# Kalyan0821/ecnf-baseline-neurips-2023

Measured on NVIDIA B200. Metric: LJ13 samples/s with exact log-q (Dopri5), higher is better.
Workload: dtype f32

## Files before the change

ecnf_b200/csrc/ecnf_solve_impl.cuh:

```cuda
#pragma once
#include <cstdio>

#include "ecnf_solve_decl.cuh"
#include "ecnf_tile.cuh"

namespace ecnf_solve_detail {

using ecnf_tile::NTHREADS;
using ecnf_tile::WCHUNK;
using ecnf_tile::ColT;
using ecnf_tile::tile_gemm;

enum { KIND_FIRST = 0, KIND_MID = 1, KIND_LAST = 2 };

static __constant__ float c_A[7][6] = {
    {0, 0, 0, 0, 0, 0},
    {(float)(1.0 / 5), 0, 0, 0, 0, 0},
    {(float)(3.0 / 40), (float)(9.0 / 40), 0, 0, 0, 0},
    {(float)(44.0 / 45), (float)(-56.0 / 15), (float)(32.0 / 9), 0, 0, 0},
    {(float)(19372.0 / 6561), (float)(-25360.0 / 2187), (float)(64448.0 / 6561), (float)(-212.0 / 729), 0, 0},
    {(float)(9017.0 / 3168), (float)(-355.0 / 33), (float)(46732.0 / 5247), (float)(49.0 / 176),
     (float)(-5103.0 / 18656), 0},
    {(float)(35.0 / 384), 0, (float)(500.0 / 1113), (float)(125.0 / 192), (float)(-2187.0 / 6784),
     (float)(11.0 / 84)}};
static __constant__ float c_C[7] = {0.f, 0.2f, 0.3f, 0.8f, (float)(8.0 / 9), 1.f, 1.f};
static __constant__ float c_BERR[7] = {(float)(35.0 / 384 - 1951.0 / 21600),
                                0.f,
                                (float)(500.0 / 1113 - 22642.0 / 50085),
                                (float)(125.0 / 192 - 451.0 / 720),
                                (float)(-2187.0 / 6784 + 12231.0 / 42400),
                                (float)(11.0 / 84 - 649.0 / 6300),
                                (float)(-1.0 / 60)};
static __constant__ float c_MID[7] = {(float)(6025192743.0 / 30085553152.0 / 2),
                               0.f,
                               (float)(51252292925.0 / 65400821598.0 / 2),
                               (float)(-2691868925.0 / 45128329728.0 / 2),
                               (float)(187940372067.0 / 1594534317056.0 / 2),
                               (float)(-1776094331.0 / 19743644256.0 / 2),
                               (float)(11237099.0 / 235043384.0 / 2)};

template <int U_, int H_>
struct Geo {
  static constexpr int U = U_, H = H_;
  static constexpr int TR = (U_ == 256) ? 64 : 128;
  static constexpr int LD = U_ + 4;
  static constexpr int RT = TR / 16;
  static constexpr int GMAX = TR / 3 + 1;
};

struct SmemLayout {
  int X1, X2, Wb, G, xt, xtacc, dacc, xs, xs0, xacc, mu, rowdot, rowsd, gv, gs1, glen, ginv, ge, tau, cvec,
      ode, red, rowslot, rowgrp, gi, gj, giz, epsv, total_floats;
};

template <int U, int H>
__host__ __device__ inline SmemLayout make_layout(int n, int dim, bool div) {
  using G_ = Geo<U, H>;
  const int D = n * dim, S = D + 1;
  SmemLayout L;
  int o = 0;
  auto take = [&](int nfl) { int r = o; o += (nfl + 3) & ~3; return r; };
  L.X1 = take(G_::TR * G_::LD);
  L.X2 = take(G_::TR * G_::LD);
  L.Wb = take(2 * WCHUNK);
  L.G = take(div ? G_::GMAX * U : 4);
  L.xt = take(div ? D * D : 4);
  L.xtacc = take(div ? D * D : 4);
  L.dacc = take(D);
  L.xs = take(D);
  L.xs0 = take(D);
  L.xacc = take(D);
  L.mu = take(4);
  L.rowdot = take(G_::TR);
  L.rowsd = take(G_::TR);
  L.gv = take(G_::TR * 3);
  L.gs1 = take(G_::TR);
  L.glen = take(G_::TR);
  L.ginv = take(G_::TR);
  L.ge = take(G_::TR);
  L.tau = take(ECNF_MAX_T);
  L.cvec = take(64);
  L.ode = take(11 * S);
  L.red = take(S + 16);
  L.rowslot = take(G_::TR);
  L.rowgrp = take(G_::TR);
  L.gi = take(G_::TR);
  L.gj = take(G_::TR);
  L.giz = take(G_::TR);
  L.epsv = take(D);
  L.total_floats = o;
  return L;
}

template <int N, int TR, int LD>
__device__ __forceinline__ void epi_act(float (&acc)[TR / 16][ColT<N>::CT], const float* __restrict__ bias,
                                        float* dst, int nrows, int r, const int* rowgrp, float* G, bool has_tan) {
  constexpr int RT = TR / 16, CT = ColT<N>::CT, NSEG = CT / 4;
  const int tid = threadIdx.x, tx = tid & 15, ty = tid >> 4, warp = tid >> 5;
  const bool active = (2 * RT * warp < nrows) && (tx * 4 < N);
  const int row0 = 2 * RT * warp + (ty & 1);
  if (active) {
#pragma unroll
    for (int rr = 0; rr < RT; ++rr) {
      const int row = row0 + 2 * rr;
      if (row >= nrows) continue;
      const int g = rowgrp[row];
      if (row != g * r) continue;
#pragma unroll
      for (int sg = 0; sg < NSEG; ++sg) {
        const int col = sg * 64 + tx * 4;
        const float4 b = *reinterpret_cast<const float4*>(bias + col);
        const float bb[4] = {b.x, b.y, b.z, b.w};
        float a[4], gg[4];
#pragma unroll
        for (int q = 0; q < 4; ++q) {
          const float z = acc[rr][4 * sg + q] + bb[q];
          const float s = ecnf_sigmoid(z);
          a[q] = z * s;
          gg[q] = s * (1.f + z * (1.f - s));
        }
        *reinterpret_cast<float4*>(dst + row * LD + col) = make_float4(a[0], a[1], a[2], a[3]);
        if (has_tan) *reinterpret_cast<float4*>(G + g * N + col) = make_float4(gg[0], gg[1], gg[2], gg[3]);
      }
    }
  }
  if (has_tan) {
    __syncthreads();
    if (active) {
#pragma unroll
      for (int rr = 0; rr < RT; ++rr) {
        const int row = row0 + 2 * rr;
        if (row >= nrows) continue;
        const int g = rowgrp[row];
        if (row == g * r) continue;
#pragma unroll
        for (int sg = 0; sg < NSEG; ++sg) {
          const int col = sg * 64 + tx * 4;
          const float4 gg = *reinterpret_cast<const float4*>(G + g * N + col);
          *reinterpret_cast<float4*>(dst + row * LD + col) =
              make_float4(acc[rr][4 * sg] * gg.x, acc[rr][4 * sg + 1] * gg.y, acc[rr][4 * sg + 2] * gg.z,
                          acc[rr][4 * sg + 3] * gg.w);
        }
      }
    }
  }
  __syncthreads();
}

template <int N, int TR, int LD>
__device__ __forceinline__ void epi_linear(float (&acc)[TR / 16][ColT<N>::CT], const float* bias, float* dst,
                                           int nrows, int r, const int* rowgrp, const float* resid) {
  constexpr int RT = TR / 16, CT = ColT<N>::CT, NSEG = CT / 4;
  const int tid = threadIdx.x, tx = tid & 15, ty = tid >> 4, warp = tid >> 5;
  const bool active = (2 * RT * warp < nrows) && (tx * 4 < N);
  const int row0 = 2 * RT * warp + (ty & 1);
  if (active) {
#pragma unroll
    for (int rr = 0; rr < RT; ++rr) {
      const int row = row0 + 2 * rr;
      if (row >= nrows) continue;
      const bool primal = (row == rowgrp[row] * r);
#pragma unroll
      for (int sg = 0; sg < NSEG; ++sg) {
        const int col = sg * 64 + tx * 4;
        float v[4] = {acc[rr][4 * sg], acc[rr][4 * sg + 1], acc[rr][4 * sg + 2], acc[rr][4 * sg + 3]};
        if (bias != nullptr && primal) {
#pragma unroll
          for (int q = 0; q < 4; ++q) v[q] += bias[col + q];
        }
        if (resid != nullptr) {
          const float4 rv = *reinterpret_cast<const float4*>(resid + row * LD + col);
          v[0] += rv.x; v[1] += rv.y; v[2] += rv.z; v[3] += rv.w;
        }
        *reinterpret_cast<float4*>(dst + row * LD + col) = make_float4(v[0], v[1], v[2], v[3]);
      }
    }
  }
  __syncthreads();
}

__device__ __forceinline__ int dirmap(int kind, int qq, int i, int j, int dim) {
  if (kind == KIND_MID) return qq;
  if (kind == KIND_LAST) return i * dim + qq;
  return (qq < dim) ? i * dim + qq : j * dim + (qq - dim);
}


template <int U, int H, bool DIV>
struct Engine {
  using G_ = Geo<U, H>;
  static constexpr int TR = G_::TR, LD = G_::LD, RT = G_::RT;
  static constexpr int NT = NTHREADS;
  const EcnfModelDev& m;
  const bool hutch;
  const int n, dim, D, ntan, ND, E;
  const int tid;
  const float* eps_g;
  float *X1, *X2, *Wb, *G, *xt, *xtacc, *dacc, *xs, *xs0, *xacc, *mu, *rowdot, *rowsd, *gv, *gs1, *glen, *ginv,
      *ge, *tau, *cvec, *ode, *red, *epsv;
  int *rowslot, *rowgrp, *gi, *gj, *giz;
  float *hA, *hB, *Ps, *Pr, *Mg;

  __device__ Engine(const EcnfModelDev& m_, float* smem, float* scratch, bool hutch_)
      : m(m_), hutch(DIV && hutch_), n(m_.n), dim(m_.dim), D(m_.n * m_.dim),
        ntan(DIV ? (hutch_ ? 1 : m_.n * m_.dim) : 0), ND(1 + ntan), E(m_.n * (m_.n - 1)), tid(threadIdx.x), eps_g(nullptr) {
    const SmemLayout L = make_layout<U, H>(n, dim, DIV);
    X1 = smem + L.X1; X2 = smem + L.X2; Wb = smem + L.Wb; G = smem + L.G; xt = smem + L.xt;
    xtacc = smem + L.xtacc; dacc = smem + L.dacc; xs = smem + L.xs; xs0 = smem + L.xs0; xacc = smem + L.xacc;
    mu = smem + L.mu; rowdot = smem + L.rowdot; rowsd = smem + L.rowsd; gv = smem + L.gv; gs1 = smem + L.gs1;
    glen = smem + L.glen; ginv = smem + L.ginv; ge = smem + L.ge; tau = smem + L.tau; cvec = smem + L.cvec;
    ode = smem + L.ode; red = smem + L.red; epsv = smem + L.epsv;
    rowslot = reinterpret_cast<int*>(smem + L.rowslot); rowgrp = reinterpret_cast<int*>(smem + L.rowgrp);
    gi = reinterpret_cast<int*>(smem + L.gi); gj = reinterpret_cast<int*>(smem + L.gj);
    giz = reinterpret_cast<int*>(smem + L.giz);
    hA = scratch; hB = hA + (size_t)n * ND * H; Ps = hB + (size_t)n * ND * H; Pr = Ps + (size_t)n * ND * U;
    Mg = Pr + (size_t)n * ND * U;
  }

  __device__ __forceinline__ void set_eps(const float* e) { eps_g = e; }
  __device__ __forceinline__ float* ode_ptr() const { return ode; }
  __device__ __forceinline__ float* red_ptr() const { return red; }

  __device__ void rowdot_tile(const float* X, const float* __restrict__ vec, int nrows) {
    const int warp = tid >> 5, lane = tid & 31;
    float v[U / 32];
#pragma unroll
    for (int j = 0; j < U / 32; ++j) v[j] = vec[lane + 32 * j];
    for (int row = warp; row < nrows; row += NTHREADS / 32) {
      float s = 0.f;
#pragma unroll
      for (int j = 0; j < U / 32; ++j) s = fmaf(X[row * LD + lane + 32 * j], v[j], s);
#pragma unroll
      for (int o = 16; o > 0; o >>= 1) s += __shfl_xor_sync(0xffffffffu, s, o);
      if (lane == 0) rowdot[row] = s;
    }
    __syncthreads();
  }

  template <int W>
  __device__ void store_node_tile(const float* X, float* dst, int node0, int nrows, int r) {
    for (int idx = tid; idx < nrows * (W / 4); idx += NTHREADS) {
      const int row = idx / (W / 4), c4 = idx % (W / 4);
      const int g = row / r, q = row - g * r;
      *reinterpret_cast<float4*>(dst + ((size_t)(node0 + g) * ND + q) * W + c4 * 4) =
          *reinterpret_cast<const float4*>(X + row * LD + c4 * 4);
    }
  }
  template <int W>
  __device__ void load_node_tile(float* X, const float* src, int node0, int nrows, int r, bool tan_valid) {
    for (int idx = tid; idx < nrows * (W / 4); idx += NTHREADS) {
      const int row = idx / (W / 4), c4 = idx % (W / 4);
      const int g = row / r, q = row - g * r;
      float4 v = make_float4(0.f, 0.f, 0.f, 0.f);
      if (q == 0 || tan_valid) v = *reinterpret_cast<const float4*>(src + ((size_t)(node0 + g) * ND + q) * W + c4 * 4);
      *reinterpret_cast<float4*>(X + row * LD + c4 * 4) = v;
    }
  }
  __device__ void set_rowgrp(int nrows, int r) {
    for (int row = tid; row < nrows; row += NTHREADS) rowgrp[row] = row / r;
  }

  __device__ void node_pre(int b, bool htan) {
    const EcnfBlockParams& bp = m.blk[b];
    if (tid < H) {
      float a = bp.bd[tid];
      for (int k = 0; k < m.T; ++k) a = fmaf(tau[k], bp.Wd[(H + k) * H + tid], a);
      cvec[tid] = a;
    }
    const int r = htan ? ND : 1;
    const int gpt = TR / r;
    for (int node0 = 0; node0 < n; node0 += gpt) {
      const int nn = min(gpt, n - node0), nrows = nn * r;
      __syncthreads();
      load_node_tile<H>(X1, hA, node0, nrows, r, true);
      set_rowgrp(nrows, r);
      __syncthreads();
      {
        float acc[RT][ColT<H>::CT];
        tile_gemm<H, H, TR, LD, true>(X1, bp.Wd, Wb, acc, nrows);
        epi_linear<H, TR, LD>(acc, cvec, X2, nrows, r, rowgrp, nullptr);
      }
      store_node_tile<H>(X2, hB, node0, nrows, r);
      {
        float acc[RT][ColT<U>::CT];
        tile_gemm<H, U, TR, LD, true>(X2, bp.We[0], Wb, acc, nrows);
        epi_linear<U, TR, LD>(acc, nullptr, X1, nrows, r, rowgrp, nullptr);
        store_node_tile<U>(X1, Ps, node0, nrows, r);
        tile_gemm<H, U, TR, LD, true>(X2, bp.We[0] + (size_t)H * U, Wb, acc, nrows);
        epi_linear<U, TR, LD>(acc, bp.be[0], X1, nrows, r, rowgrp, nullptr);
        store_node_tile<U>(X1, Pr, node0, nrows, r);
      }
    }
    __syncthreads();
  }

  __device__ void node_post(int b, bool htan) {
    const EcnfBlockParams& bp = m.blk[b];
    const int r = ND;
    const int gpt = TR / r;
    for (int node0 = 0; node0 < n; node0 += gpt) {
      const int nn = min(gpt, n - node0), nrows = nn * r;
      __syncthreads();
      load_node_tile<U>(X1, Mg, node0, nrows, r, true);
      load_node_tile<H>(X2, hB, node0, nrows, r, htan);
      set_rowgrp(nrows, r);
      __syncthreads();
      {
        float acc[RT][ColT<U>::CT];
        tile_gemm<U, U, TR, LD, true>(X1, bp.Wh[0], Wb, acc, nrows);
        tile_gemm<H, U, TR, LD, false>(X2, bp.Wh[0] + (size_t)U * U, Wb, acc, nrows);
        epi_act<U, TR, LD>(acc, bp.bh[0], X1, nrows, r, rowgrp, G, DIV);
        for (int l = 1; l < m.L; ++l) {
          tile_gemm<U, U, TR, LD, true>(X1, bp.Wh[l], Wb, acc, nrows);
          epi_act<U, TR, LD>(acc, bp.bh[l], X1, nrows, r, rowgrp, G, DIV);
        }
      }
      {
        float acc[RT][ColT<H>::CT];
        tile_gemm<U, H, TR, LD, true>(X1, bp.Wh[m.L], Wb, acc, nrows);
        epi_linear<H, TR, LD>(acc, bp.bh[m.L], X1, nrows, r, rowgrp, X2);
      }
      store_node_tile<H>(X1, hA, node0, nrows, r);
    }
    __syncthreads();
  }

  __device__ void edge_phase(int b, int kind, bool htan, bool lastb) {
    const EcnfBlockParams& bp = m.blk[b];
    const int nact = !DIV ? 0 : (kind == KIND_MID ? ntan : kind == KIND_LAST ? dim : 2 * dim);
    const int r = 1 + nact;
    const int gpt = DIV ? min(TR / r, n - 1) : TR;
    const float inv_sqrt_nb = rsqrtf((float)(n - 1));
    const float* wd = bp.We[0] + (size_t)2 * H * U;
    const float bpv = bp.bp[0];
    const float bav = bp.ba[0];
    for (int i = tid; i < D; i += NTHREADS) { xacc[i] = 0.f; dacc[i] = 0.f; }
    if (DIV && kind != KIND_LAST)
      for (int i = tid; i < D * ntan; i += NTHREADS) xtacc[i] = 0.f;
    if (!lastb)
      for (int i = tid; i < n * ND * U; i += NTHREADS) Mg[i] = 0.f;
    __syncthreads();

    int e0 = 0;
    while (e0 < E) {
      int ng;
      if (DIV) {
        const int i = e0 / (n - 1);
        ng = min(gpt, (i + 1) * (n - 1) - e0);
      } else {
        ng = min(TR, E - e0);
      }
      const int nrows = ng * r;
      if (tid < ng) {
        const int e = e0 + tid, i = e / (n - 1), jj = e - i * (n - 1);
        int j = i + 1 + jj; if (j >= n) j -= n;
        float s = 0.f;
        for (int c = 0; c < dim; ++c) {
          const float v = xs[i * dim + c] - xs[j * dim + c];
          gv[tid * 3 + c] = v;
          s = fmaf(v, v, s);
        }
        const int isz = (s == 0.f);
        const float s1 = isz ? 1.f : s;
        const float len = sqrtf(s1);
        gi[tid] = i; gj[tid] = j; giz[tid] = isz; gs1[tid] = s1; glen[tid] = len; ginv[tid] = 1.f / (m.C + len);
      }
      __syncthreads();
      for (int row = tid; row < nrows; row += NTHREADS) {
        const int g = row / r, q = row - g * r;
        rowgrp[row] = g;
        if (q == 0) {
          rowslot[row] = 0;
          rowsd[row] = gs1[g];
        } else {
          const int i = gi[g], j = gj[g];
          const int k = dirmap(kind, q - 1, i, j, dim);
          float sd = 0.f;
          for (int c = 0; c < dim; ++c)
            sd = fmaf(gv[g * 3 + c], xt[(i * dim + c) * ntan + k] - xt[(j * dim + c) * ntan + k], sd);
          rowslot[row] = 1 + k;
          rowsd[row] = giz[g] ? 0.f : 2.f * sd;
        }
      }
      __syncthreads();
      {
        const int col = tid % U;
        const float wdc = wd[col];
        for (int g = tid / U; g < ng; g += NTHREADS / U) {
          const int row = g * r;
          const float z = Ps[((size_t)gj[g] * ND) * U + col] + Pr[((size_t)gi[g] * ND) * U + col] + rowsd[row] * wdc;
          const float s = ecnf_sigmoid(z);
          X1[row * LD + col] = z * s;
          if (DIV) G[g * U + col] = s * (1.f + z * (1.f - s));
        }
        if (DIV) {
          __syncthreads();
          for (int row = tid / U; row < nrows; row += NTHREADS / U) {
            const int g = rowgrp[row];
            if (row == g * r) continue;
            float z = rowsd[row] * wdc;
            if (htan) {
              const int slot = rowslot[row];
              z += Ps[((size_t)gj[g] * ND + slot) * U + col] + Pr[((size_t)gi[g] * ND + slot) * U + col];
            }
            X1[row * LD + col] = z * G[g * U + col];
          }
        }
      }
      __syncthreads();
      {
        float acc[RT][ColT<U>::CT];
        for (int l = 1; l < m.L; ++l) {
          tile_gemm<U, U, TR, LD, true>(X1, bp.We[l], Wb, acc, nrows);
          epi_act<U, TR, LD>(acc, bp.be[l], X1, nrows, r, rowgrp, G, DIV);
        }
        if (!lastb) {
          rowdot_tile(X1, bp.wa, nrows);
          if (tid < ng) ge[tid] = ecnf_sigmoid(rowdot[tid * r] + bav);
          __syncthreads();
          for (int idx = tid; idx < nrows * U; idx += NTHREADS) {
            const int row = idx / U, col = idx - row * U;
            const int g = rowgrp[row];
            const float e = ge[g];
            float v = X1[row * LD + col] * e;
            if (row != g * r) v = fmaf(X1[g * r * LD + col], e * (1.f - e) * rowdot[row], v);
            X2[row * LD + col] = v;
          }
          __syncthreads();
          if (DIV) {
            const int i = gi[0];
            for (int idx = tid; idx < r * U; idx += NTHREADS) {
              const int q = idx / U, col = idx - q * U;
              const bool shared_q = (q == 0) || kind == KIND_MID || (q - 1 < dim);
              if (shared_q) {
                const int slot = (q == 0) ? 0 : 1 + dirmap(kind, q - 1, i, 0, dim);
                float s = 0.f;
                for (int g = 0; g < ng; ++g) s += X2[(g * r + q) * LD + col];
                Mg[((size_t)i * ND + slot) * U + col] += s * inv_sqrt_nb;
              } else {
                for (int g = 0; g < ng; ++g) {
                  const int slot = 1 + gj[g] * dim + (q - 1 - dim);
                  Mg[((size_t)i * ND + slot) * U + col] += X2[(g * r + q) * LD + col] * inv_sqrt_nb;
                }
              }
            }
          } else {
            const int i_first = e0 / (n - 1), i_last = (e0 + ng - 1) / (n - 1);
            for (int idx = tid; idx < (i_last - i_first + 1) * U; idx += NTHREADS) {
              const int ri = idx / U, col = idx - ri * U, i = i_first + ri;
              const int ga = max(e0, i * (n - 1)) - e0, gb = min(e0 + ng, (i + 1) * (n - 1)) - e0;
              float s = 0.f;
              for (int g = ga; g < gb; ++g) s += X2[g * LD + col];
              Mg[(size_t)i * U + col] += s * inv_sqrt_nb;
            }
          }
        }
        for (int l = 0; l < m.L; ++l) {
          tile_gemm<U, U, TR, LD, true>(X1, bp.Wx[l], Wb, acc, nrows);
          epi_act<U, TR, LD>(acc, bp.bx[l], X1, nrows, r, rowgrp, G, DIV);
        }
      }
      rowdot_tile(X1, bp.wp, nrows);
      {
        const int i_first = e0 / (n - 1), i_last = (e0 + ng - 1) / (n - 1);
        const int nprim = (i_last - i_first + 1) * dim;
        const int nwork_tan = DIV ? (r - 1) * dim : 0;
        for (int idx = tid; idx < nprim + nwork_tan; idx += NTHREADS) {
          if (idx < nprim) {
            const int ri = idx / dim, c = idx - ri * dim, i = i_first + ri;
            const int ga = max(e0, i * (n - 1)) - e0, gb = min(e0 + ng, (i + 1) * (n - 1)) - e0;
            float s = 0.f;
            for (int g = ga; g < gb; ++g) s = fmaf((rowdot[g * r] + bpv) * gv[g * 3 + c], ginv[g], s);
            xacc[i * dim + c] += s;
          } else {
            const int t2 = idx - nprim;
            const int q = 1 + t2 / dim, c = t2 % dim;
            const int i = gi[0];
            for (int g = 0; g < ng; ++g) {
              const int j = gj[g];
              const int k = dirmap(kind, q - 1, i, j, dim);
              if (kind == KIND_LAST && k != i * dim + c) continue;
              const float pg = rowdot[g * r] + bpv, pd = rowdot[g * r + q];
              const float vc = gv[g * 3 + c], inv = ginv[g];
              const float vd = xt[(i * dim + c) * ntan + k] - xt[(j * dim + c) * ntan + k];
              const float ld = giz[g] ? 0.f : rowsd[g * r + q] / (2.f * glen[g]);
              const float cd = (pd * vc + pg * vd) * inv - pg * vc * ld * inv * inv;
              if (kind == KIND_LAST) dacc[i * dim + c] += cd;
              else xtacc[(i * dim + c) * ntan + k] += cd;
            }
          }
        }
      }
      __syncthreads();
      e0 += ng;
    }
  }

  __device__ void eval(float t, const float* xin, const int32_t* feat, float* fout) {
    if (tid < dim) {
      float s = 0.f;
      for (int i = 0; i < n; ++i) s += xin[i * dim + tid];
      mu[tid] = s / (float)n;
    }
    if (tid >= 32 && tid < 32 + m.T / 2) {
      const int k = tid - 32;
      const float arg = (t * 1000.f) * m.freqs[k];
      tau[k] = sinf(arg);
      tau[k + m.T / 2] = cosf(arg);
    }
    __syncthreads();
    for (int i = tid; i < D; i += NTHREADS) {
      const float v = xin[i] - mu[i % dim];
      xs[i] = v;
      xs0[i] = v;
    }
    if (DIV && !hutch) {
      const float invn = 1.f / (float)n;
      for (int idx = tid; idx < D * D; idx += NTHREADS) {
        const int a = idx / D, k = idx - a * D;
        const int ia = a / dim, ca = a - ia * dim, ik = k / dim, ck = k - ik * dim;
        xt[idx] = (ca == ck) ? ((ia == ik ? 1.f : 0.f) - invn) : 0.f;
      }
    }
    if (hutch) {
      for (int i = tid; i < D; i += NTHREADS) epsv[i] = eps_g[i];
      __syncthreads();
      for (int i = tid; i < D; i += NTHREADS) {
        float mean = 0.f;
        for (int node = 0; node < n; ++node) mean += epsv[node * dim + i % dim];
        xt[i] = epsv[i] - mean / (float)n;
      }
    }
    for (int idx = tid; idx < n * H; idx += NTHREADS) {
      const int node = idx / H, col = idx - node * H;
      int f = feat[node];
      f = max(0, min(m.nfeat - 1, f));
      hA[(size_t)node * ND * H + col] = m.embed[f * H + col];
    }
    __syncthreads();
    for (int b = 0; b < m.nblocks; ++b) {
      const bool last = (b == m.nblocks - 1);
      const int kind = hutch ? KIND_MID : (last ? KIND_LAST : (b == 0 ? KIND_FIRST : KIND_MID));
      const bool htan = DIV && b > 0;
      node_pre(b, htan);
      edge_phase(b, kind, htan, last);
      if (!last) node_post(b, htan);
      const float invnb = 1.f / (float)(n - 1);
      for (int i = tid; i < D; i += NTHREADS) xs[i] += xacc[i] * invnb;
      if (DIV && (!last || hutch))
        for (int i = tid; i < D * ntan; i += NTHREADS) xt[i] += xtacc[i] * invnb;
      __syncthreads();
    }
    const float fs = m.final_scaling[0];
    for (int i = tid; i < D; i += NTHREADS) fout[i] = (xs[i] - xs0[i] - mu[i % dim]) * fs;
    if (DIV && tid == 0) {
      float s = 0.f;
      if (hutch) {
        for (int d = 0; d < D; ++d) s = fmaf(epsv[d], xt[d] - epsv[d], s);
        fout[D] = fs * s;
      } else {
        const float invnb = 1.f / (float)(n - 1);
        for (int d = 0; d < D; ++d) s += xt[d * D + d] + dacc[d] * invnb;
        fout[D] = fs * (s - (float)D);
      }
    }
    __syncthreads();
  }
};

__device__ __forceinline__ float clip_to_end(float tprev, float tnext, float T1, bool keep) {
  if (tnext > T1 - 1e-6f) return keep ? T1 : tprev + 0.5f * (T1 - tprev);
  return tnext;
}

template <class Eng, bool DIV, bool SAVE>
__device__ __forceinline__ void solve_body(const KernelArgs& a, Eng& eng, long long& s_traj, float* s_ctl) {
  const int tid = threadIdx.x;
  const int D = eng.D, S = DIV ? D + 1 : D;
  float* y = eng.ode_ptr();
  float* ys = y + S;
  float* f0 = ys + S;
  float* fo = f0 + S;
  float* kk = fo + S;
  float* red = eng.red_ptr();
  const ecnf_solve_ctrl& c = a.ctrl;
  const bool vf_mode = (a.mode == ECNF_MODE_VF || a.mode == ECNF_MODE_VF_DIV);
  const bool reverse = (a.mode == ECNF_MODE_LOGPROB);
  const float dir = reverse ? -1.f : 1.f;
  const float T0 = reverse ? -1.f : 0.f, T1 = reverse ? 0.f : 1.f;
  enum { PH_VF = 0, PH_F0 = 1, PH_F1 = 2, PH_STAGE = 3 };

  auto rms_of_red = [&]() -> float {
    __syncthreads();
    if (tid == 0) {
      float s = 0.f;
      for (int i = 0; i < S; ++i) s = fmaf(red[i], red[i], s);
      s_ctl[0] = sqrtf(s / (float)S);
    }
    __syncthreads();
    const float r = s_ctl[0];
    __syncthreads();
    return r;
  };
  auto base_logp = [&](const float* v) -> float {
    __syncthreads();
    if (tid == 0) {
      float s = 0.f;
      for (int cdim = 0; cdim < eng.dim; ++cdim) {
        float mean = 0.f;
        for (int i = 0; i < eng.n; ++i) mean += v[i * eng.dim + cdim] / a.m.base_scale;
        mean /= (float)eng.n;
        for (int i = 0; i < eng.n; ++i) {
          const float z = v[i * eng.dim + cdim] / a.m.base_scale - mean;
          s = fmaf(z, z, s);
        }
      }
      const float dof = (float)((eng.n - 1) * eng.dim);
      s_ctl[1] = -0.5f * s - 0.5f * dof * 1.8378770664093453f - dof * logf(a.m.base_scale);
    }
    __syncthreads();
    const float r = s_ctl[1];
    __syncthreads();
    return r;
  };

  for (;;) {
    if (tid == 0) s_traj = (long long)atomicAdd(a.counter, 1u);
    __syncthreads();
    const long long b = s_traj;
    __syncthreads();
    if (b >= a.B) break;
    const int32_t* feat = a.feat + b * eng.n;
    const float* xin = a.x_init + b * D;
    eng.set_eps(a.eps ? a.eps + b * D : nullptr);
    auto put = [&](int k, int i, float v) {
      if (i < D) a.out_traj[(b * a.n_save + k) * D + i] = v;
      else a.out_traj_delta[b * a.n_save + k] = v;
    };
    int next_save = 0;

    int phase, stage = 0, n_steps = 0, n_acc = 0, n_evals = 0, status = 0;
    float tprev = T0, tnext = T0, dt = 0.f, h0 = 0.f, d1 = 0.f, t_eval, lp0_start = 0.f;
    bool at_dtmin = false;
    const float* ein;
    if (vf_mode) {
      for (int i = tid; i < D; i += Eng::NT) ys[i] = xin[i];
      phase = PH_VF;
      t_eval = a.t_in[b];
      ein = ys;
    } else {
      for (int i = tid; i < S; i += Eng::NT) y[i] = (i < D) ? xin[i] : 0.f;
      phase = PH_F0;
      t_eval = dir * T0;
      ein = y;
    }
    __syncthreads();
    if constexpr (SAVE) {
      for (; next_save < a.n_save && a.ts[next_save] <= T0; ++next_save)
        for (int i = tid; i < S; i += Eng::NT) put(next_save, i, y[i]);
    }
    if (DIV && !vf_mode && !reverse) lp0_start = base_logp(y);

    bool running = true;
    while (running) {
      eng.eval(t_eval, ein, feat, fo);
      ++n_evals;
      bool begin_step = false;
      if (phase == PH_VF) {
        for (int i = tid; i < D; i += Eng::NT) a.out_x[b * D + i] = fo[i];
        if (DIV && tid == 0) a.out_logs[b] = fo[D];
        running = false;
      } else if (phase == PH_F0) {
        for (int i = tid; i < S; i += Eng::NT) f0[i] = dir * fo[i];
        __syncthreads();
        if (c.fixed) {
          tnext = clip_to_end(tprev, tprev + fabsf(c.step_size), T1, true);
          begin_step = true;
        } else {
          for (int i = tid; i < S; i += Eng::NT) red[i] = y[i] / (c.atol + fabsf(y[i]) * c.rtol);
          const float d0 = rms_of_red();
          for (int i = tid; i < S; i += Eng::NT) red[i] = f0[i] / (c.atol + fabsf(y[i]) * c.rtol);
          d1 = rms_of_red();
          const bool cond = (d0 < 1e-5f) || (d1 < 1e-5f);
          h0 = cond ? 1e-6f : 0.01f * d0 / d1;
          for (int i = tid; i < S; i += Eng::NT) ys[i] = y[i] + h0 * f0[i];
          __syncthreads();
          t_eval = dir * (tprev + h0);
          ein = ys;
          phase = PH_F1;
        }
      } else if (phase == PH_F1) {
        for (int i = tid; i < S; i += Eng::NT) red[i] = (dir * fo[i] - f0[i]) / (c.atol + fabsf(y[i]) * c.rtol);
        const float d2 = rms_of_red() / h0;
        const float md = fmaxf(d1, d2);
        const float h1 = (md <= 1e-15f) ? fmaxf(1e-6f, h0 * 1e-3f) : powf(0.01f / md, 1.f / c.error_order);
        const float dt0 = fmaxf(fminf(100.f * h0, h1), c.dtmin);
        tnext = clip_to_end(tprev, tprev + dt0, T1, true);
        begin_step = true;
      } else {
        for (int i = tid; i < S; i += Eng::NT) kk[stage * S + i] = (dir * fo[i]) * dt;
        __syncthreads();
        if (stage < 6) {
          ++stage;
        } else {
          bool keep = true;
          float new_prev, new_next;
          if (c.fixed) {
            new_prev = tnext;
            new_next = tnext + dt;
          } else {
            for (int i = tid; i < S; i += Eng::NT) {
              float e = 0.f;
              for (int j = 0; j < 7; ++j) {
                const float bj = c_BERR[j];
                if (bj != 0.f) e = e + bj * kk[j * S + i];
              }
              red[i] = (c.err_scale * e) / (c.atol + fmaxf(fabsf(y[i]), fabsf(ys[i])) * c.rtol);
            }
            const float err = rms_of_red();
            keep = (err < 1.f) || at_dtmin;
            const float inv = (err == 0.f) ? INFINITY : 1.f / err;
            float factor = c.safety * powf(inv, 1.f / c.error_order);
            const float fmin_ = keep ? 1.f : c.factormin;
            factor = fminf(fmaxf(factor, fmin_), c.factormax);
            float ndt = dt * factor;
            at_dtmin = ndt <= c.dtmin;
            ndt = fmaxf(ndt, c.dtmin);
            new_prev = keep ? tnext : tprev;
            new_next = new_prev + ndt;
          }
          new_prev = fminf(new_prev, T1);
          new_next = clip_to_end(new_prev, new_next, T1, keep);
          if constexpr (SAVE) {
            for (; keep && next_save < a.n_save && a.ts[next_save] <= tnext; ++next_save) {
              const float tau_s = a.ts[next_save];
              const bool at_end = !(tau_s < tnext);
              const float sx = (tau_s - tprev) / dt;
              for (int i = tid; i < S; i += Eng::NT) {
                const float y0 = y[i], y1 = ys[i];
                float v = y1;
                if (!at_end) {
                  const float k0 = kk[i], k6 = kk[6 * S + i];
                  float ym = y0;
                  for (int j = 0; j < 7; ++j) {
                    const float cj = c_MID[j];
                    if (cj != 0.f) ym = ym + cj * kk[j * S + i];
                  }
                  const float pa = 2.f * (k6 - k0) - 8.f * (y1 + y0) + 16.f * ym;
                  const float pb = 5.f * k0 - 3.f * k6 + 18.f * y0 + 14.f * y1 - 32.f * ym;
                  const float pc = k6 - 4.f * k0 - 11.f * y0 - 5.f * y1 + 16.f * ym;
                  v = (((pa * sx + pb) * sx + pc) * sx + k0) * sx + y0;
                }
                put(next_save, i, v);
              }
            }
          }
          if (keep) {
            for (int i = tid; i < S; i += Eng::NT) { y[i] = ys[i]; f0[i] = dir * fo[i]; }
            ++n_acc;
          }
          __syncthreads();
          tprev = new_prev;
          tnext = new_next;
          ++n_steps;
          if (!(tprev < T1)) running = false;
          else if (n_steps >= c.max_steps) { status = 1; running = false; }
          else begin_step = true;
        }
      }
      if (begin_step) {
        dt = tnext - tprev;
        for (int i = tid; i < S; i += Eng::NT) kk[i] = f0[i] * dt;
        __syncthreads();
        stage = 1;
        phase = PH_STAGE;
        if (c.max_steps <= 0) { status = 1; running = false; }
      }
      if (running && phase == PH_STAGE) {
        for (int i = tid; i < S; i += Eng::NT) {
          float v = y[i];
          for (int j = 0; j < stage; ++j) {
            const float aj = c_A[stage][j];
            if (aj != 0.f) v = v + aj * kk[j * S + i];
          }
          ys[i] = v;
        }
        __syncthreads();
        t_eval = dir * (tprev + c_C[stage] * dt);
        ein = ys;
      }
    }
    if (vf_mode) { __syncthreads(); continue; }
    if constexpr (SAVE) {
      const int left = a.n_save - next_save;
      for (int idx = tid; idx < left * S; idx += Eng::NT) put(next_save + idx / S, idx % S, __int_as_float(0x7fffffff));
    }

    for (int i = tid; i < D; i += Eng::NT) a.out_x[b * D + i] = y[i];
    float lpb_end = 0.f;
    if (DIV && reverse) lpb_end = base_logp(y);
    if (tid == 0) {
      if (a.out_stats) {
        a.out_stats[b * 4 + 0] = n_steps; a.out_stats[b * 4 + 1] = n_acc;
        a.out_stats[b * 4 + 2] = n_evals; a.out_stats[b * 4 + 3] = status;
      }
      if (DIV && a.out_logs) {
        const float delta = y[D];
        if (!reverse) {
          a.out_logs[b * 3 + 0] = lp0_start - delta;
          a.out_logs[b * 3 + 1] = lp0_start;
          a.out_logs[b * 3 + 2] = delta;
        } else {
          a.out_logs[b * 3 + 0] = lpb_end + delta;
          a.out_logs[b * 3 + 1] = lpb_end;
          a.out_logs[b * 3 + 2] = delta;
        }
      }
    }
    __syncthreads();
  }
}

template <int U, int H, bool DIV, bool SAVE>
__global__ void __launch_bounds__(NTHREADS, 1) ecnf_solve_kernel(const __grid_constant__ KernelArgs a) {
  extern __shared__ __align__(16) float smem[];
  __shared__ long long s_traj;
  __shared__ float s_ctl[8];
  Engine<U, H, DIV> eng(a.m, smem, a.scratch + (size_t)blockIdx.x * a.scratch_stride, a.eps != nullptr);
  solve_body<Engine<U, H, DIV>, DIV, SAVE>(a, eng, s_traj, s_ctl);
}

template <int U, int H, bool DIV>
int simt_check(const ecnf_model* mdl) {
  const SmemLayout L = make_layout<U, H>(mdl->cfg.n_frames, mdl->cfg.dim, DIV);
  const size_t smem = (size_t)L.total_floats * sizeof(float);
  if (smem > 227 * 1024) {
    ecnf_set_error("shared memory need %zu B exceeds 227 KB (n_frames=%d dim=%d U=%d)", smem, mdl->cfg.n_frames,
                   mdl->cfg.dim, U);
    return ECNF_ERR_UNSUPPORTED;
  }
  if (DIV && 1 + mdl->cfg.n_frames * mdl->cfg.dim > Geo<U, H>::TR) {
    ecnf_set_error("1 + n_frames*dim = %d tangent slots exceed the %d-row tile of U=%d", 1 + mdl->cfg.n_frames * mdl->cfg.dim,
                   Geo<U, H>::TR, U);
    return ECNF_ERR_UNSUPPORTED;
  }
  return ECNF_OK;
}

template <int U, int H, bool DIV, bool SAVE>
int launch_t(const ecnf_model* mdl, KernelArgs& a, int grid, cudaStream_t st) {
  const int rc = simt_check<U, H, DIV>(mdl);
  if (rc != ECNF_OK) return rc;
  const size_t smem = (size_t)make_layout<U, H>(mdl->cfg.n_frames, mdl->cfg.dim, DIV).total_floats * sizeof(float);
  auto kern = ecnf_solve_kernel<U, H, DIV, SAVE>;
  ECNF_CHECK_CUDA(cudaFuncSetAttribute(kern, cudaFuncAttributeMaxDynamicSharedMemorySize, (int)smem));
  kern<<<grid, NTHREADS, smem, st>>>(a);
  ECNF_CHECK_CUDA(cudaGetLastError());
  return ECNF_OK;
}


}
```

ecnf_b200/csrc/ecnf_solve_tc.cuh:

```cuda
#pragma once
#include "ecnf_solve_impl.cuh"
#include "ecnf_tc.cuh"

namespace ecnf_solve_detail {

using namespace ecnf_tc;

constexpr int TC_NT = 384;
constexpr int TC_EPI = 256, TC_SIDE = 96;
#ifndef TC_WPREFETCH
#define TC_WPREFETCH 0
#endif
constexpr int TC_BOP = 65536;
constexpr uint32_t TC_LBO = 128, TC_SBO = 2048;
constexpr uint32_t TC_LBO_K = 2048, TC_SBO_K = 128;
constexpr int TC_WCOL = 256;

constexpr uint32_t CH_VALID = 1u << 31, CH_GRPEND = 1u << 22, CH_OWNER = 1u << 23, CH_RUNEND = 1u << 24;
__host__ __device__ __forceinline__ int ch_gid(uint32_t w) { return (int)(w & 1023u); }
__host__ __device__ __forceinline__ int ch_qb(uint32_t w) { return (int)((w >> 10) & 255u); }
__host__ __device__ __forceinline__ int ch_cnt(uint32_t w) { return (int)((w >> 18) & 15u); }
enum { TH_N = 0, TH_FLUSH, TH_WIN_I, TH_WIN_NR, TH_WIN_S, TH_WIN_NS, TH_NCH , TH_IFIRST = 10, TH_ILAST, TH_P, TH_MR, TH_RUNMASK };

__device__ __forceinline__ float fast_sigmoid(float z) {
  float e, r;
  asm("ex2.approx.ftz.f32 %0, %1;" : "=f"(e) : "f"(z * -1.4426950408889634f));
  asm("rcp.approx.ftz.f32 %0, %1;" : "=f"(r) : "f"(1.f + e));
  return r;
}
__device__ __forceinline__ float2 fast_sigmoid2(float2 z) {
  const float2 t = mul2(z, splat2(-1.4426950408889634f));
  float2 e, r;
  asm("ex2.approx.ftz.f32 %0, %1;" : "=f"(e.x) : "f"(t.x));
  asm("ex2.approx.ftz.f32 %0, %1;" : "=f"(e.y) : "f"(t.y));
  const float2 d = add2(splat2(1.f), e);
  asm("rcp.approx.ftz.f32 %0, %1;" : "=f"(r.x) : "f"(d.x));
  asm("rcp.approx.ftz.f32 %0, %1;" : "=f"(r.y) : "f"(d.y));
  return r;
}
__device__ __forceinline__ float2 col2(const float (&v)[64], int c) { return make_float2(v[c], v[c + 1]); }
__device__ __forceinline__ void set_col2(float (&v)[64], int c, float2 p) { v[c] = p.x; v[c + 1] = p.y; }

__host__ __device__ inline int tc_rows_of_kind(int kind, int n, int dim, int ntan) {
  const int ND = 1 + ntan;
  return (kind == TT_NODE1 || kind == TT_EDGE1) ? 1 : kind == TT_NODE ? ND : kind == TT_FIRST ? 1 + 2 * dim : kind == TT_MID ? ND : 1 + dim;
}

__host__ __device__ inline int tc_pack(int kind, int n, int dim, int SUB, int MR, uint32_t* out, int ntan, uint32_t* stage = nullptr) {
  const int ND = 1 + ntan, nb = n - 1;
  const bool edge = kind >= TT_FIRST;
  const int ngroups = edge ? n * nb : n;
  const int r = tc_rows_of_kind(kind, n, dim, ntan);
  const bool dense = (r == 1);
  const int CAP = 16 * SUB;
  int tile = 0, p = 0;
  int win_i = 0, win_nr = 0, win_s = 0, win_ns = 0, i_first = 0, i_last = 0;
  int run_start = 0;
  auto tp = [&](int t) { return stage ? stage : out + (size_t)t * TC_TILE_WORDS; };
  auto word_index = [&](int q) { return (q % SUB) * 16 + ((q / SUB) % 2) * 8 + q / (2 * SUB); };
  auto end_run = [&](bool each_chunk = false) {
    if (out && p > run_start) {
      tp(tile)[word_index(p - 1)] |= CH_RUNEND;
      for (int q = run_start; q < p; ++q)
        if (each_chunk || q + 2 * SUB >= p) tp(tile)[word_index(q)] |= CH_GRPEND;
    }
    run_start = p;
  };
  auto close = [&](int flush) {
    if (p == 0) return;
    end_run();
    if (out) {
      uint32_t* h = tp(tile) + 32;
      int nmax0 = 0, nmax1 = 0;
      for (int sb = 0; sb < SUB; ++sb)
        for (int hh = 0; hh < 2; ++hh) {
          const int first = sb + SUB * hh;
          const int cntp = p > first ? (p - first + 2 * SUB - 1) / (2 * SUB) : 0;
          h[TH_NCH + sb * 2 + hh] = (uint32_t)cntp;
          if (hh == 0 && cntp > nmax0) nmax0 = cntp;
          if (hh == 1 && cntp > nmax1) nmax1 = cntp;
        }
      int N = nmax1 > 0 ? 64 + 8 * nmax1 : 8 * nmax0;
      N = (N + 15) & ~15;
      h[TH_N] = (uint32_t)(N < 16 ? 16 : N);
      h[TH_FLUSH] = (uint32_t)flush;
      h[TH_WIN_I] = (uint32_t)win_i; h[TH_WIN_NR] = (uint32_t)win_nr; h[TH_WIN_S] = (uint32_t)win_s; h[TH_WIN_NS] = (uint32_t)win_ns;
      h[TH_IFIRST] = (uint32_t)i_first; h[TH_ILAST] = (uint32_t)i_last; h[TH_P] = (uint32_t)p; h[TH_MR] = (uint32_t)MR;
      uint32_t rm = 0u;
      for (int q = 0; q < p; ++q)
        if (tp(tile)[word_index(q)] & CH_RUNEND) rm |= 1u << q;
      h[TH_RUNMASK] = rm;
      if (stage)
        for (int k = 0; k < TC_TILE_WORDS; ++k) out[(size_t)tile * TC_TILE_WORDS + k] = stage[k];
    }
    ++tile;
    p = 0; run_start = 0;
  };
  auto put = [&](int gid, int qb, int cnt, bool owner) {
    if (p == CAP) close(0);
    if (p == 0 && out)
      for (int k = 0; k < TC_TILE_WORDS; ++k) tp(tile)[k] = 0;
    const int i = edge ? gid / nb : gid;
    if (p == 0) i_first = i;
    i_last = edge ? (gid + (dense ? cnt - 1 : 0)) / nb : gid + (dense ? cnt - 1 : 0);
    if (out)
      tp(tile)[word_index(p)] = CH_VALID | (uint32_t)gid | ((uint32_t)qb << 10) | ((uint32_t)cnt << 18) | (owner ? CH_OWNER : 0u);
    ++p;
  };
  if (dense) {
    win_i = 0; win_nr = n; win_s = 0; win_ns = 1;
    for (int g = 0; g < ngroups; g += 8) {
      put(g, 0, ngroups - g < 8 ? ngroups - g : 8, true);
      end_run();
    }
    close(kind == TT_EDGE1 ? 1 : 0);
    return tile;
  }
  if (kind == TT_NODE) {
    for (int g = 0; g < n; ++g)
      for (int qb = 1; qb < r; qb += 7) { put(g, qb, 1 + (r - qb < 7 ? r - qb : 7), qb == 1); end_run(); }
    close(0);
    return tile;
  }
  if (kind == TT_LAST) {
    for (int i = 0; i < n; ++i) {
      for (int e = i * nb; e < (i + 1) * nb; ++e) {
        if (p == CAP) close(0);
        put(e, 1, r, true);
      }
      end_run();
    }
    close(0);
    return tile;
  }
  if (kind == TT_FIRST) {
    const int rows_per = 1 + dim;
    int W = MR / rows_per; if (W < 1) W = 1; if (W > n) W = n;
    for (int i0 = 0; i0 < n; i0 += W) {
      win_i = i0; win_nr = (n - i0 < W) ? n - i0 : W; win_s = 0; win_ns = rows_per;
      for (int i = i0; i < i0 + win_nr; ++i) {
        for (int e = i * nb; e < (i + 1) * nb; ++e) {
          if (p == CAP) { end_run(true); close(0); }
          put(e, 1, r, true);
        }
        end_run(true);
      }
      close(1);
    }
    return tile;
  }
  if (ND <= MR) {
    int W = MR / ND; if (W > n) W = n;
    for (int i0 = 0; i0 < n; i0 += W) {
      win_i = i0; win_nr = (n - i0 < W) ? n - i0 : W; win_s = 0; win_ns = ND;
      for (int i = i0; i < i0 + win_nr; ++i)
        for (int qb = 1; qb < r; qb += 7) {
          for (int e = i * nb; e < (i + 1) * nb; ++e) {
            if (p == CAP) close(0);
            put(e, qb, 1 + (r - qb < 7 ? r - qb : 7), qb == 1);
          }
          end_run();
        }
      close(1);
    }
  } else {
    const int cpw = (MR - 1) / 7 > 0 ? (MR - 1) / 7 : 1;
    for (int i = 0; i < n; ++i)
      for (int qw = 1; qw < r; qw += 7 * cpw) {
        const int q_end = (qw + 7 * cpw < r) ? qw + 7 * cpw : r;
        win_i = i; win_nr = 1; win_s = (qw == 1) ? 0 : qw; win_ns = q_end - win_s;
        for (int qb = qw; qb < q_end; qb += 7) {
          for (int e = i * nb; e < (i + 1) * nb; ++e) {
            if (p == CAP) close(0);
            put(e, qb, 1 + (r - qb < 7 ? r - qb : 7), qb == 1);
          }
          end_run();
        }
        close(1);
      }
  }
  return tile;
}

template <int U, int H>
__host__ __device__ inline TcSmemLayout make_tc_layout(int n, int dim, int MR) {
  constexpr int SUB = 128 / U;
  const int D = n * dim, S = D + 1, E = n * (n - 1);
  TcSmemLayout L;
  int o = 0;
  auto take = [&](int bytes) { int r = o; o += (bytes + 127) & ~127; return r; };
  L.bop = take(2 * TC_BOP);
  L.mrows = MR;
  L.macc = take(2 * SUB * (MR + 1) * U * 4);
  L.xt = take(D * D * 4);
  L.xtacc = take(D * D * 4);
  L.dacc = take(D * 4);
  L.xs = take(D * 4);
  L.xs0 = take(D * 4);
  L.xacc = take(D * 4);
  L.mu = take(16);
  L.tau = take(ECNF_MAX_T * 4);
  L.cvec = take(64 * 4);
  L.ode = take(11 * S * 4);
  L.red = take((S + 16) * 4);
  L.colsd = take(4 * SUB * 128 * 4);
  L.colmrow = take(4 * SUB * 128 * 4);
  L.chw = take(4 * 32 * 4);
  L.hdr = take(4 * 16 * 4);
  L.pdot = take(2 * 8 * 64 * 4);
  L.pdh = take(4 * 8 * 64 * 4);
  L.wA = take(8 * 64 * 4);
  L.wB = take(8 * 64 * 4);
  L.cdbuf = take(SUB * 128 * 3 * 4);
  L.egv = take(E * 4 * 4);
  L.bars = take(128);
  L.prof = take(32 * 8);
  L.total_bytes = o;
  return L;
}
template <int U, int H>
__host__ inline int tc_pick_mrows(int n, int dim, bool div) {
  const int ND = div ? 1 + n * dim : 1;
  if (!div) return n;
  int best = 0;
  const int cap = ND > 40 ? ND : 40;
  for (int mr = 8; mr <= cap; ++mr) {
    if (mr < ND && (mr - 1) % 7 != 0) continue;
    if (make_tc_layout<U, H>(n, dim, mr).total_bytes + 1024 <= 227 * 1024) best = mr;
  }
  return best;
}

extern __shared__ __align__(1024) unsigned char smem_tc[];

#define TCF(field) (reinterpret_cast<float*>(smem_tc + a.lay.field))
#define TCI(field) (reinterpret_cast<int*>(smem_tc + a.lay.field))
#define TCW(field) (reinterpret_cast<uint32_t*>(smem_tc + a.lay.field))

template <int U_, int H_, bool DIV>
struct EngineTC {
  static constexpr int U = U_, H = H_, SUB = 128 / U_;
  static constexpr int NT = TC_NT;
  static constexpr int KN = SUB * H;
  static constexpr int ROWB = 4 * H;
  const KernelArgs& a;
  const EcnfModelDev& m;
  const TcImages& img;
  const bool hutch;
  const int n, dim, D, ntan, ND, E;
  const float* eps_g;
  const int tid, f, hh, warp, lane, sub, fu;
  const bool is_epi, is_side;
  uint32_t tmem;
  uint32_t lane_addr;
  uint32_t par;

  enum { B_READY = 0, B_DONE = 1, B_BUILT = 2, B_HEADS = 3, B_BFREE = 4 };
  enum { P_NODE_PRE, P_EDGE, P_NODE_POST, P_WAIT, P_EPI, P_MSG, P_HEAD, P_WLOAD, P_SIDE_WAIT, P_SIDE_GATHER, P_SIDE_COORD,
         P_SIDE_META, P_SIDE_CPWAIT, P_NBUILD, P_NCOUNT };
#ifdef ECNF_TC_PROFILE
  long long prof_t0, prof_t1;
  __device__ __forceinline__ long long* prof_s() const { return reinterpret_cast<long long*>(smem_tc + a.lay.prof); }
  __device__ __forceinline__ void pbeg() { prof_t0 = clock64(); }
  __device__ __forceinline__ void pend(int k) { const long long t1 = clock64(); if (tid == 0) prof_s()[k] += t1 - prof_t0; prof_t0 = t1; }
  __device__ __forceinline__ void qbeg() { prof_t1 = clock64(); }
  __device__ __forceinline__ void qend(int k) { const long long t1 = clock64(); if (tid == 0 || tid == TC_EPI) prof_s()[k] += t1 - prof_t1; prof_t1 = t1; }
#else
  __device__ __forceinline__ void pbeg() {}
  __device__ __forceinline__ void pend(int) {}
  __device__ __forceinline__ void qbeg() {}
  __device__ __forceinline__ void qend(int) {}
#endif

  __device__ __forceinline__ void set_eps(const float* e) { eps_g = e; }
  __device__ __forceinline__ float* ode_ptr() const { return TCF(ode); }
  __device__ __forceinline__ float* red_ptr() const { return TCF(red); }
  __device__ __forceinline__ uint64_t* bar(int kind, int s) const { return reinterpret_cast<uint64_t*>(smem_tc + a.lay.bars) + kind * 2 + s; }
  __device__ __forceinline__ uint32_t* tmem_slot() const { return reinterpret_cast<uint32_t*>(smem_tc + a.lay.bars + 96); }
  __device__ __forceinline__ float* hA() const { return a.scratch + (size_t)blockIdx.x * a.scratch_stride; }
  __device__ __forceinline__ float* hB() const { return hA() + (size_t)n * ND * H; }
  __device__ __forceinline__ float* Mg() const { return hB() + (size_t)n * ND * H; }
  __device__ __forceinline__ float* Ph() const { return Mg() + (size_t)n * ND * U; }
  __device__ __forceinline__ unsigned char* Himg() const { return reinterpret_cast<unsigned char*>(Ph() + (size_t)n * ND * U); }

  __device__ __forceinline__ EngineTC(const KernelArgs& a_)
      : a(a_), m(a_.m), img(a_.img), hutch(DIV && a_.eps != nullptr), n(a_.m.n), dim(a_.m.dim), D(a_.m.n * a_.m.dim),
        ntan(DIV ? (a_.eps != nullptr ? 1 : a_.m.n * a_.m.dim) : 0), ND(1 + (DIV ? (a_.eps != nullptr ? 1 : a_.m.n * a_.m.dim) : 0)),
        E(a_.m.n * (a_.m.n - 1)), eps_g(nullptr), tid(threadIdx.x), f(threadIdx.x & 127), hh((threadIdx.x >> 7) & 1), warp(threadIdx.x >> 5),
        lane(threadIdx.x & 31), sub((threadIdx.x & 127) / U_), fu((threadIdx.x & 127) % U_), is_epi(threadIdx.x < TC_EPI),
        is_side(threadIdx.x >= TC_EPI && threadIdx.x < TC_EPI + TC_SIDE) {
    if (tid == 0) {
      mbar_init(bar(B_READY, 0), TC_EPI); mbar_init(bar(B_READY, 1), TC_EPI);
      mbar_init(bar(B_DONE, 0), 1); mbar_init(bar(B_DONE, 1), 1);
      mbar_init(bar(B_BUILT, 0), TC_SIDE); mbar_init(bar(B_BUILT, 1), TC_SIDE);
      mbar_init(bar(B_HEADS, 0), TC_EPI); mbar_init(bar(B_HEADS, 1), TC_EPI);
      mbar_init(bar(B_BFREE, 0), 1); mbar_init(bar(B_BFREE, 1), 1);
#ifdef ECNF_TC_PROFILE
      for (int k = 0; k < P_NCOUNT; ++k) prof_s()[k] = 0;
#endif
    }
    __syncwarp();
    if (warp == 0) tmem_alloc(tmem_slot(), 512);
    tc_fence_before();
    __syncthreads();
    tc_fence_after();
    tmem = *tmem_slot();
    lane_addr = (uint32_t)(32 * (warp & 3)) << 16;
    par = 0;
    if (is_epi) {
      uint32_t z[32];
#pragma unroll
      for (int c = 0; c < 32; ++c) z[c] = 0u;
#pragma unroll
      for (int q = 0; q < 4; ++q) tmem_st32(tmem + lane_addr + 128u * hh + 32u * q, z);
      tmem_wait_st();
    }
    if (is_side)
      for (int k = tid - TC_EPI; k < ROWB / 4; k += TC_SIDE) reinterpret_cast<uint32_t*>(Himg() + (size_t)n * ND * ROWB)[k] = 0u;
    tc_fence_before();
    __syncthreads();
    tc_fence_after();
  }
  __device__ __forceinline__ void finish(long long* out) {
#ifdef ECNF_TC_PROFILE
    if (out && tid == 0 && blockIdx.x == 0)
      for (int k = 0; k < P_NCOUNT; ++k) out[k] = prof_s()[k];
#endif
    tc_fence_before();
    __syncthreads();
    if (warp == 0) tmem_dealloc(tmem, 512);
  }

  __device__ __forceinline__ void epi_bar() const { named_bar_sync(1, TC_EPI); }
  __device__ __forceinline__ void half_bar() const { named_bar_sync(2 + hh, TC_EPI / 2); }
  __device__ __forceinline__ void side_bar() const { named_bar_sync(4, TC_SIDE); }
  __device__ __forceinline__ void phase_bar() const { named_bar_sync(5, TC_EPI + TC_SIDE); }
  __device__ __forceinline__ void wait_bar(int kind, int s) {
    const uint32_t bit = 1u << (kind * 2 + s);
    mbar_wait_parked(bar(kind, s), (par & bit) ? 1u : 0u, 20000u);
    par ^= bit;
    tc_fence_after();
  }
  __device__ __forceinline__ void wait_done(int s) { qbeg(); wait_bar(B_DONE, s); qend(P_WAIT); }
  __device__ __forceinline__ void arrive(int kind, int s) {
    fence_proxy_async();
    tc_fence_before();
    mbar_arrive(bar(kind, s));
  }
  __device__ __forceinline__ void issue_mma(int s, int tb, int wait_kind, uint32_t a_col, int K, bool kmajor, bool free_b,
                                            bool drained = false) {
    if (lane == 0) {
      if (drained) wait_bar(B_READY, s);
      wait_bar(wait_kind, s);
      const int N = hdr(tb, TH_N);
      const uint32_t idesc = make_idesc_bf16(128, N) | (kmajor ? 0u : IDESC_B_MN);
      const uint32_t bsm = smem_u32(smem_tc + a.lay.bop) + (uint32_t)s * TC_BOP;
      const uint32_t lbo = kmajor ? TC_LBO_K : TC_LBO, sbo = kmajor ? TC_SBO_K : TC_SBO;
      uint64_t bh = make_sdesc(bsm, lbo, sbo);
      uint64_t bl = make_sdesc(bsm + 32768u, lbo, sbo);
      const uint32_t acc = tmem + 128u * s;
      uint32_t a_hi = tmem + a_col, a_lo = tmem + a_col + (uint32_t)(K >> 1);
      const int nk = K >> 4;
      mma_ts(acc, a_hi, bh, idesc, 0u);
      mma_ts(acc, a_lo, bh, idesc, 1u);
      mma_ts(acc, a_hi, bl, idesc, 1u);
      for (int ks = 1; ks < nk; ++ks) {
        bh += (2u * lbo) >> 4; bl += (2u * lbo) >> 4; a_hi += 8; a_lo += 8;
        mma_ts(acc, a_hi, bh, idesc, 1u);
        mma_ts(acc, a_lo, bh, idesc, 1u);
        mma_ts(acc, a_hi, bl, idesc, 1u);
      }
      mma_commit(bar(B_DONE, s));
      if (free_b) mma_commit(bar(B_BFREE, s));
    }
  }

  __device__ __forceinline__ uint32_t my_acc(int s) const { return tmem + 128u * s + lane_addr + 64u * hh; }
  __device__ __forceinline__ void ld_acc(int s, float (&v)[64]) {
    uint32_t x[32], y[32];
    const uint32_t addr = my_acc(s);
    tmem_ld32(addr, x);
    tmem_ld32(addr + 32u, y);
    tmem_wait_ld();
#pragma unroll
    for (int c = 0; c < 32; ++c) { v[c] = __uint_as_float(x[c]); v[32 + c] = __uint_as_float(y[c]); }
  }
  __device__ __forceinline__ void write_B(int s, const float (&v)[64], int krow) {
    unsigned char* base = smem_tc + a.lay.bop + s * TC_BOP + (8 * hh) * (int)TC_SBO + krow * 16;
#pragma unroll
    for (int g8 = 0; g8 < 8; ++g8) {
      uint32_t h[4], l[4];
#pragma unroll
      for (int p = 0; p < 4; ++p) split_pack(v[8 * g8 + 2 * p], v[8 * g8 + 2 * p + 1], h[p], l[p]);
      *reinterpret_cast<uint4*>(base + g8 * (int)TC_SBO) = make_uint4(h[0], h[1], h[2], h[3]);
      *reinterpret_cast<uint4*>(base + 32768 + g8 * (int)TC_SBO) = make_uint4(l[0], l[1], l[2], l[3]);
    }
  }
  __device__ __forceinline__ void ld_half_issue(int s, int hf, uint32_t (&x)[32]) { tmem_ld32(my_acc(s) + 32u * hf, x); }
  template <bool L0>
  __device__ __forceinline__ void act_half(float (&v)[64], int hf, float bias, int tb, float wdf) {
    const float* sdp = TCF(colsd) + (tb * SUB + sub) * 128 + 64 * hh;
#pragma unroll
    for (int c4 = 0; c4 < 4; ++c4) act_chunk<L0>(v, 4 * hf + c4, bias, sdp, wdf);
  }
  __device__ __forceinline__ void write_half(int s, const float (&v)[64], int hf, int krow) {
    unsigned char* base = smem_tc + a.lay.bop + s * TC_BOP + (8 * hh + 4 * hf) * (int)TC_SBO + krow * 16;
#pragma unroll
    for (int g8 = 0; g8 < 4; ++g8) {
      uint32_t h[4], l[4];
#pragma unroll
      for (int p = 0; p < 4; ++p) split_pack(v[32 * hf + 8 * g8 + 2 * p], v[32 * hf + 8 * g8 + 2 * p + 1], h[p], l[p]);
      *reinterpret_cast<uint4*>(base + g8 * (int)TC_SBO) = make_uint4(h[0], h[1], h[2], h[3]);
      *reinterpret_cast<uint4*>(base + 32768 + g8 * (int)TC_SBO) = make_uint4(l[0], l[1], l[2], l[3]);
    }
  }
  __device__ __forceinline__ static int tb_of(int s, int tile) { return s * 2 + ((tile >> 1) & 1); }
  __device__ __forceinline__ int hdr(int tb, int k) const { return TCI(hdr)[tb * 16 + k]; }
  __device__ __forceinline__ int my_nch(int tb) const { return hdr(tb, TH_NCH + sub * 2 + hh); }
  __device__ __forceinline__ uint32_t my_chw(int tb, int ch) const { return TCW(chw)[tb * 32 + sub * 16 + 8 * hh + ch]; }
  template <bool L0>
  __device__ __forceinline__ void act_rule(float (&v)[64], float bias, int tb, float wdf) {
    const float* sdp = TCF(colsd) + (tb * SUB + sub) * 128 + 64 * hh;
#pragma unroll
    for (int ch = 0; ch < 8; ++ch) act_chunk<L0>(v, ch, bias, sdp, wdf);
  }
  template <bool L0>
  __device__ __forceinline__ static void act_chunk(float (&v)[64], int ch, float bias, const float* sdp, float wdf) {
    const int c0 = 8 * ch;
    if constexpr (L0) {
      const float4 s0 = reinterpret_cast<const float4*>(sdp)[2 * ch], s1 = reinterpret_cast<const float4*>(sdp)[2 * ch + 1];
      const float2 w2 = splat2(wdf);
      set_col2(v, c0, fma2(make_float2(s0.x, s0.y), w2, col2(v, c0)));
      set_col2(v, c0 + 2, fma2(make_float2(s0.z, s0.w), w2, col2(v, c0 + 2)));
      set_col2(v, c0 + 4, fma2(make_float2(s1.x, s1.y), w2, col2(v, c0 + 4)));
      set_col2(v, c0 + 6, fma2(make_float2(s1.z, s1.w), w2, col2(v, c0 + 6)));
    }
    if constexpr (!DIV) {
#pragma unroll
      for (int u = 0; u < 8; u += 2) {
        const float2 z = add2(col2(v, c0 + u), splat2(bias));
        set_col2(v, c0 + u, mul2(z, fast_sigmoid2(z)));
      }
    } else {
      const float z = v[c0] + bias;
      const float sg = fast_sigmoid(z);
      const float cur = sg * (1.f + z * (1.f - sg));
      set_col2(v, c0, mul2(make_float2(z, v[c0 + 1]), make_float2(sg, cur)));
#pragma unroll
      for (int u = 2; u < 8; u += 2) set_col2(v, c0 + u, mul2(col2(v, c0 + u), splat2(cur)));
    }
  }
  template <int W>
  __device__ __forceinline__ void bfly_round(float (&x)[32]) const {
    const bool b = (lane & (W >> 1)) != 0;
#pragma unroll
    for (int i = 0; i < W; ++i) {
      const float keep = b ? x[W + i] : x[i], send = b ? x[i] : x[W + i];
      x[i] = keep + __shfl_xor_sync(0xffffffffu, send, W >> 1);
    }
  }
  __device__ __forceinline__ void warp_dot(const float (&v)[64], float wf, float* pd) {
    float x[32];
    {
      const bool b = (lane & 16) != 0;
      const float2 w2 = splat2(wf);
#pragma unroll
      for (int i = 0; i < 32; i += 2) {
        const float2 lo2 = mul2(col2(v, i), w2), hi2 = mul2(col2(v, 32 + i), w2);
        const float lo[2] = {lo2.x, lo2.y}, hi[2] = {hi2.x, hi2.y};
#pragma unroll
        for (int j = 0; j < 2; ++j) {
          const float keep = b ? hi[j] : lo[j], send = b ? lo[j] : hi[j];
          x[i + j] = keep + __shfl_xor_sync(0xffffffffu, send, 16);
        }
      }
    }
    bfly_round<16>(x);
    bfly_round<8>(x);
    bfly_round<4>(x);
    bfly_round<2>(x);
    *reinterpret_cast<float2*>(pd + 2 * lane) = make_float2(x[0], x[1]);
  }
  __device__ __forceinline__ float full_dot(const float* pd, int h2, int sb, int c) const {
    const float* p4 = pd + (4 * h2) * 64 + c;
    if constexpr (SUB == 1) return (p4[0] + p4[64]) + (p4[128] + p4[192]);
    else return p4[(2 * sb) * 64] + p4[(2 * sb + 1) * 64];
  }
  template <int K>
  __device__ __forceinline__ void fetch_w(int img_off, uint32_t (&wv)[2][K / 4]) {
    constexpr int NC = K / 16;
    const uint4* src = reinterpret_cast<const uint4*>(img.base + img_off);
#pragma unroll
    for (int p = 0; p < 2; ++p)
#pragma unroll
      for (int j = 0; j < NC; ++j) {
        const uint4 q = __ldg(src + (size_t)(p * (K / 8) + hh * NC + j) * 128 + f);
        wv[p][4 * j] = q.x; wv[p][4 * j + 1] = q.y; wv[p][4 * j + 2] = q.z; wv[p][4 * j + 3] = q.w;
      }
  }
  template <int K>
  __device__ __forceinline__ void store_w(const uint32_t (&wv)[2][K / 4], uint32_t col) {
#pragma unroll
    for (int p = 0; p < 2; ++p) {
      const uint32_t addr = tmem + col + lane_addr + (uint32_t)(p * (K / 2) + hh * (K / 4));
      if constexpr (K == 128) tmem_st32(addr, wv[p]);
      else tmem_st16(addr, wv[p]);
    }
    tmem_wait_st();
  }
  template <int K>
  __device__ __forceinline__ void load_w(int img_off, uint32_t col) {
    constexpr int NC = K / 16;
    uint32_t wv[2][K / 4];
    const uint4* src = reinterpret_cast<const uint4*>(img.base + img_off);
#pragma unroll
    for (int p = 0; p < 2; ++p)
#pragma unroll
      for (int j = 0; j < NC; ++j) {
        const uint4 q = __ldg(src + (size_t)(p * (K / 8) + hh * NC + j) * 128 + f);
        wv[p][4 * j] = q.x; wv[p][4 * j + 1] = q.y; wv[p][4 * j + 2] = q.z; wv[p][4 * j + 3] = q.w;
      }
#pragma unroll
    for (int p = 0; p < 2; ++p) {
      const uint32_t addr = tmem + col + lane_addr + (uint32_t)(p * (K / 2) + hh * (K / 4));
      if constexpr (K == 128) tmem_st32(addr, wv[p]);
      else tmem_st16(addr, wv[p]);
    }
    tmem_wait_st();
  }

  __device__ __forceinline__ const uint32_t* tile_ptr(int kind, int tile) const {
    return a.tabs.base + (size_t)(a.tabs.off[kind] + tile) * TC_TILE_WORDS;
  }
  __device__ __forceinline__ bool col_of(uint32_t cw, int c, int& gid, int& q) const {
    const int u = c & 7;
    const bool valid = (cw & CH_VALID) && u < ch_cnt(cw);
    const int qb = ch_qb(cw);
    if (qb == 0) { gid = ch_gid(cw) + u; q = 0; }
    else { gid = ch_gid(cw); q = (u == 0) ? 0 : qb + u - 1; }
    return valid;
  }

  template <class P>
  __device__ __forceinline__ void run_phase(P& p) {
    const int ntiles = p.ntiles, NL = p.NL;
    const int npairs = (ntiles + 1) >> 1;
    const int total_q = npairs * NL;
    if (is_epi || (P::side_build && is_side)) p.prologue();
    if (is_epi && p.stream) {
      load_w<128>(p.wimg(0), TC_WCOL);
      if (total_q > 1) load_w<128>(p.wimg(1 % NL), TC_WCOL + 128);
    }
    if constexpr (P::side_build) {
      if (is_epi || is_side) phase_bar();
    }
    if (is_side) {
      if constexpr (P::side_build) {
#pragma unroll 1
        for (int t0 = 0; t0 < 2 && t0 < ntiles; ++t0) {
          p.side_meta(tb_of(t0, t0), t0);
          p.side_gather(t0, t0);
          cp_async_wait<0>();
          arrive(B_BUILT, t0);
        }
#pragma unroll 1
        for (int t0 = 2; t0 < 4 && t0 < ntiles; ++t0) p.side_meta(tb_of(t0 & 1, t0), t0);
#pragma unroll 1
        for (int pr = 0; pr < npairs; ++pr) {
          qbeg();
#pragma unroll 1
          for (int s = 0; s < 2; ++s) {
            const int tile = 2 * pr + s, ntile = tile + 2;
            if (tile >= ntiles) continue;
            if (ntile < ntiles) {
              wait_bar(B_BFREE, s);
              qend(P_SIDE_WAIT);
              p.side_gather(s, ntile);
              qend(P_SIDE_GATHER);
              cp_async_wait<0>();
              qend(P_SIDE_CPWAIT);
            }
            wait_bar(B_HEADS, s);
            qend(P_SIDE_WAIT);
            if (ntile < ntiles) arrive(B_BUILT, s);
          }
#pragma unroll 1
          for (int s = 0; s < 2; ++s) {
            const int tile = 2 * pr + s;
            if (tile >= ntiles) continue;
            p.side_coords(tb_of(s, tile), tile);
            qend(P_SIDE_COORD);
            if (tile + 4 < ntiles) p.side_meta(tb_of(s, tile + 4), tile + 4);
            qend(P_SIDE_META);
          }
        }
      }
      return;
    }
    const int first_kind = P::side_build ? B_BUILT : B_READY;
#pragma unroll 1
    for (int s = 0; s < 2; ++s) {
      if (s >= ntiles) continue;
      if (is_epi) {
        if constexpr (!P::side_build) { p.build(s, tb_of(s, s), s); arrive(B_READY, s); }
      } else {
        issue_mma(s, tb_of(s, s), first_kind, p.a_col(0, 0), p.K(0), P::side_build, false);
      }
    }
    int q = 0;
#pragma unroll 1
    for (int pr = 0; pr < npairs; ++pr) {
#pragma unroll 1
      for (int w = 0; w < NL; ++w, ++q) {
#pragma unroll 1
        for (int s = 0; s < 2; ++s) {
          const int tile = 2 * pr + s;
          if (tile >= ntiles) continue;
          const bool last_slot = (s == 1) || (tile + 1 >= ntiles);
          const int ntile = tile + 2;
          const int tb = tb_of(s, tile);
          if (is_epi) {
            const bool do_w = p.stream && last_slot && q + 2 < total_q;
#if TC_WPREFETCH
            uint32_t wv[2][32];
            if (do_w) fetch_w<128>(p.wimg((w + 2) % NL), wv);
            wait_done(s);
            if (do_w) { qbeg(); store_w<128>(wv, TC_WCOL + 128 * (q & 1)); qend(P_WLOAD); }
#else
            wait_done(s);
            if (do_w) { qbeg(); load_w<128>(p.wimg((w + 2) % NL), TC_WCOL + 128 * (q & 1)); qend(P_WLOAD); }
#endif
            p.epi(s, tb, tile, w);
            if (w < NL - 1) arrive(B_READY, s);
            else if constexpr (P::side_build) arrive(B_HEADS, s);
            else if (ntile < ntiles) { p.build(s, tb_of(s, ntile), ntile); arrive(B_READY, s); }
          } else {
            if (w < NL - 1)
              issue_mma(s, tb, B_READY, p.a_col(q + 1, w + 1), p.K(w + 1), false, P::side_build && w + 1 == NL - 1 && ntile < ntiles);
            else if (ntile < ntiles)
              issue_mma(s, tb_of(s, ntile), first_kind, p.a_col(q + 1, 0), p.K(0), P::side_build, false, P::side_build);
          }
        }
      }
    }
  }

  __device__ __forceinline__ void node_meta(int tb, int kind, int tile) {
    epi_bar();
    const uint32_t* tp = tile_ptr(kind, tile);
    if (tid < 128) {
#pragma unroll
      for (int sb = 0; sb < SUB; ++sb) {
        const uint32_t cw = __ldg(tp + sb * 16 + (tid >> 3));
        int g, q;
        const bool valid = col_of(cw, tid, g, q);
        TCI(colmrow)[(tb * SUB + sb) * 128 + tid] = valid ? g * ND + q : -1;
      }
    } else if (tid < 128 + 48) {
      const uint32_t w = __ldg(tp + (tid - 128));
      if (tid < 128 + 32) TCW(chw)[tb * 32 + (tid - 128)] = w;
      else TCW(hdr)[tb * 16 + (tid - 160)] = w;
    }
    epi_bar();
  }

  struct NodePre {
    EngineTC& e;
    int b, ntiles, NL, kind;
    static constexpr bool stream = false;
    static constexpr bool side_build = false;
    __device__ __forceinline__ uint32_t a_col(int, int w) const { return TC_WCOL + 64u * w; }
    __device__ __forceinline__ int K(int) const { return KN; }
    __device__ __forceinline__ int wimg(int) const { return 0; }
    __device__ __forceinline__ void prologue() {
      const KernelArgs& a = e.a;
      const EcnfBlockParams& bp = e.m.blk[b];
      const TcImgBlock& ib = e.img.blk[b];
      if (e.tid < H) {
        float cv = bp.bd[e.tid];
        for (int k = 0; k < e.m.T; ++k) cv = fmaf(TCF(tau)[k], bp.Wd[(H + k) * H + e.tid], cv);
        TCF(cvec)[e.tid] = cv;
      }
      e.template load_w<KN>(ib.Wd, TC_WCOL);
      if (NL > 1) e.template load_w<KN>(ib.Wh0h, TC_WCOL + 64);
    }
    __device__ __forceinline__ void build(int s, int tb, int tile) {
      const KernelArgs& a = e.a;
      e.qbeg();
      e.node_meta(tb, kind, tile);
      if (e.fu < H) {
        float v[64];
        const float* src = e.hA() + e.fu;
        const int* ro_ = TCI(colmrow) + (tb * SUB + e.sub) * 128 + 64 * e.hh;
#pragma unroll
        for (int c = 0; c < 64; ++c) {
          const int ro = ro_[c];
          const float x = src[(size_t)(ro >= 0 ? ro : 0) * H];
          v[c] = ro >= 0 ? x : 0.f;
        }
        e.write_B(s, v, e.sub * H + e.fu);
      }
      e.qend(P_NBUILD);
    }
    __device__ __forceinline__ void epi(int s, int tb, int, int w) {
      const KernelArgs& a = e.a;
      const EcnfBlockParams& bp = e.m.blk[b];
      float v[64];
      e.ld_acc(s, v);
      const int* ro_ = TCI(colmrow) + (tb * SUB + e.sub) * 128 + 64 * e.hh;
      if (w == 0) {
        if (e.fu >= H) return;
        const float bias = TCF(cvec)[e.fu];
        float* dst = e.hB() + e.fu;
        unsigned char* himg = e.Himg() + 2 * e.fu;
        const bool dense = (kind == TT_NODE1);
#pragma unroll
        for (int c = 0; c < 64; ++c) {
          const bool pr = dense || (c & 7) == 0;
          v[c] += pr ? bias : 0.f;
          const int ro = ro_[c];
          if (ro >= 0) {
            dst[(size_t)ro * H] = v[c];
            const __nv_bfloat16 hi = __float2bfloat16_rn(v[c]);
            const __nv_bfloat16 lo = __float2bfloat16_rn(v[c] - __bfloat162float(hi));
            *reinterpret_cast<__nv_bfloat16*>(himg + (size_t)ro * ROWB) = hi;
            *reinterpret_cast<__nv_bfloat16*>(himg + (size_t)ro * ROWB + 2 * H) = lo;
          }
        }
        if (NL > 1) e.write_B(s, v, e.sub * H + e.fu);
      } else {
        const float bias = bp.bh[0][e.fu];
        float* dst = e.Ph() + e.fu;
        const bool dense = (kind == TT_NODE1);
#pragma unroll
        for (int c = 0; c < 64; ++c) {
          const bool pr = dense || (c & 7) == 0;
          const int ro = ro_[c];
          if (ro >= 0) dst[(size_t)ro * U] = v[c] + (pr ? bias : 0.f);
        }
      }
    }
  };

  struct NodePost {
    EngineTC& e;
    int b, ntiles, NL, kind;
    bool htan;
    static constexpr bool stream = true;
    static constexpr bool side_build = false;
    __device__ __forceinline__ uint32_t a_col(int q, int) const { return TC_WCOL + 128u * (q & 1); }
    __device__ __forceinline__ int K(int) const { return 128; }
    __device__ __forceinline__ void prologue() {}
    __device__ __forceinline__ int wimg(int w) const {
      const TcImgBlock& ib = e.img.blk[b];
      const int L = e.m.L;
      return w == 0 ? ib.Wh0m : (w < L ? ib.Wh[w] : ib.WhL);
    }
    __device__ __forceinline__ void build(int s, int tb, int tile) {
      const KernelArgs& a = e.a;
      e.qbeg();
      e.node_meta(tb, kind, tile);
      float v[64];
      const float* src = e.Mg() + e.fu;
      const int* ro_ = TCI(colmrow) + (tb * SUB + e.sub) * 128 + 64 * e.hh;
#pragma unroll
      for (int cb = 0; cb < 64; cb += 16) {
#pragma unroll
        for (int u = 0; u < 16; ++u) {
          const int ro = ro_[cb + u];
          const float x = src[(size_t)(ro >= 0 ? ro : 0) * U];
          v[cb + u] = ro >= 0 ? x : 0.f;
        }
      }
      e.write_B(s, v, e.f);
      e.qend(P_NBUILD);
    }
    __device__ __forceinline__ void epi(int s, int tb, int, int w) {
      const KernelArgs& a = e.a;
      const EcnfBlockParams& bp = e.m.blk[b];
      const int L = e.m.L;
      const int* ro_ = TCI(colmrow) + (tb * SUB + e.sub) * 128 + 64 * e.hh;
      float v[64];
      if (w == 0) {
        const float* ph = e.Ph() + e.fu;
        e.ld_acc(s, v);
#pragma unroll
        for (int cb = 0; cb < 64; cb += 16) {
          float pv[16];
#pragma unroll
          for (int u = 0; u < 16; ++u) {
            const int c = cb + u;
            const bool pr = DIV ? ((c & 7) == 0) : true;
            const int ro = ro_[c];
            const bool use = ro >= 0 && (pr || htan);
            const float x = ph[(size_t)(use ? ro : 0) * U];
            pv[u] = use ? x : 0.f;
          }
#pragma unroll
          for (int u = 0; u < 16; ++u) v[cb + u] += pv[u];
        }
        e.template act_rule<false>(v, 0.f, tb, 0.f);
        e.write_B(s, v, e.f);
      } else if (w < L) {
        const float bias = bp.bh[w][e.fu];
        e.ld_acc(s, v);
        e.template act_rule<false>(v, bias, tb, 0.f);
        e.write_B(s, v, e.f);
      } else {
        if (e.fu >= H) return;
        const float bias = bp.bh[L][e.fu];
        const float* hin = e.hB() + e.fu;
        float* dst = e.hA() + e.fu;
        e.ld_acc(s, v);
#pragma unroll
        for (int cb = 0; cb < 64; cb += 16) {
          float hv[16];
#pragma unroll
          for (int u = 0; u < 16; ++u) {
            const int c = cb + u;
            const bool pr = DIV ? ((c & 7) == 0) : true;
            const int ro = ro_[c];
            const bool use = ro >= 0 && (pr || htan);
            const float x = hin[(size_t)(use ? ro : 0) * H];
            hv[u] = (use ? x : 0.f) + (pr ? bias : 0.f);
          }
#pragma unroll
          for (int u = 0; u < 16; ++u) {
            const int ro = ro_[cb + u];
            if (ro >= 0) dst[(size_t)ro * H] = v[cb + u] + hv[u];
          }
        }
      }
    }
  };

  struct EdgePh {
    EngineTC& e;
    int b, ntiles, NL, kind;
    bool htan, want_msg;
    float wdf, waf, wpf;
    static constexpr bool stream = true;
    static constexpr bool side_build = true;
    __device__ __forceinline__ uint32_t a_col(int q, int) const { return TC_WCOL + 128u * (q & 1); }
    __device__ __forceinline__ int K(int) const { return 128; }
    __device__ __forceinline__ int ekind() const { return kind == TT_FIRST ? KIND_FIRST : kind == TT_MID ? KIND_MID : KIND_LAST; }
    __device__ __forceinline__ int wimg(int w) const {
      const TcImgBlock& ib = e.img.blk[b];
      const int L = e.m.L;
      return w == 0 ? ib.We0 : (w < L ? ib.We[w] : ib.Wx[w - L]);
    }
    __device__ __forceinline__ void prologue() {
      const KernelArgs& a = e.a;
      const EcnfBlockParams& bp = e.m.blk[b];
      const int n = e.n, dim = e.dim, D = e.D;
      constexpr int NTH = TC_EPI + TC_SIDE;
      if (e.is_epi) {
        wdf = bp.We[0][(size_t)2 * H * U + e.fu];
        waf = bp.wa[e.fu];
        wpf = bp.wp[e.fu];
      }
      for (int i = e.tid; i < D; i += NTH) { TCF(xacc)[i] = 0.f; TCF(dacc)[i] = 0.f; }
      if (DIV && kind != TT_LAST)
        for (int i = e.tid; i < D * e.ntan; i += NTH) TCF(xtacc)[i] = 0.f;
      if (want_msg)
        for (int i = e.tid; i < 2 * SUB * (a.lay.mrows + 1) * U; i += NTH) TCF(macc)[i] = 0.f;
      for (int ed = e.tid; ed < e.E; ed += NTH) {
        const int i = ed / (n - 1), jj = ed - i * (n - 1);
        int j = i + 1 + jj; if (j >= n) j -= n;
        float vv[3];
        for (int c = 0; c < 3; ++c) vv[c] = c < dim ? TCF(xs)[i * dim + c] - TCF(xs)[j * dim + c] : 0.f;
        reinterpret_cast<float4*>(TCF(egv))[ed] = make_float4(vv[0], vv[1], vv[2], __int_as_float(i | (j << 8)));
      }
    }
    __device__ __forceinline__ float4 edge_geo(int ed, int& i, int& j, float& sq) const {
      const KernelArgs& a = e.a;
      const float4 g = reinterpret_cast<const float4*>(TCF(egv))[ed];
      const int ij = __float_as_int(g.w);
      i = ij & 255; j = ij >> 8;
      sq = fmaf(g.z, g.z, fmaf(g.y, g.y, g.x * g.x));
      return g;
    }

    __device__ __forceinline__ void side_gather(int s, int tile) {
      const KernelArgs& a = e.a;
      const int n = e.n, ND = e.ND;
      const uint32_t* tp = e.tile_ptr(kind, tile);
      const unsigned char* himg = e.Himg();
#pragma unroll 1
      for (int item = e.tid - TC_EPI; item < SUB * 128; item += TC_SIDE) {
        const int sb = item >> 7, c = item & 127;
        unsigned char* bbase = smem_tc + a.lay.bop + s * TC_BOP + (c >> 3) * (int)TC_SBO_K + (c & 7) * 16;
        const uint32_t cw = __ldg(tp + sb * 16 + (c >> 3));
        int ed, q;
        const bool valid = e.col_of(cw, c, ed, q);
        int rs = n * ND, rr = n * ND;
        if (valid && (q == 0 || htan)) {
          const int ij = __float_as_int(TCF(egv)[ed * 4 + 3]);
          const int i = ij & 255, j = ij >> 8;
          const int slot = q == 0 ? 0 : 1 + dirmap(ekind(), q - 1, i, j, e.dim);
          rs = j * ND + slot; rr = i * ND + slot;
        }
        const unsigned char* src_s = himg + (size_t)rs * ROWB;
        const unsigned char* src_r = himg + (size_t)rr * ROWB;
        unsigned char* d0 = bbase + ((sb * 2 * H) >> 3) * (int)TC_LBO_K;
#pragma unroll
        for (int g = 0; g < H / 8; ++g) {
          cp_async16(d0 + g * (int)TC_LBO_K, src_s + 16 * g);
          cp_async16(d0 + 32768 + g * (int)TC_LBO_K, src_s + 2 * H + 16 * g);
          cp_async16(d0 + (H / 8 + g) * (int)TC_LBO_K, src_r + 16 * g);
          cp_async16(d0 + 32768 + (H / 8 + g) * (int)TC_LBO_K, src_r + 2 * H + 16 * g);
        }
      }
      cp_async_commit();
    }
    __device__ __forceinline__ void side_meta(int tb, int tile) {
      const KernelArgs& a = e.a;
      const int sc = e.tid - TC_EPI, n = e.n, dim = e.dim, D = e.D, ND = e.ND;
      const uint32_t* tp = e.tile_ptr(kind, tile);
      const int win_i = (int)__ldg(tp + 32 + TH_WIN_I), win_s = (int)__ldg(tp + 32 + TH_WIN_S), win_ns = (int)__ldg(tp + 32 + TH_WIN_NS);
      const int dump = a.lay.mrows * U;
#pragma unroll 1
      for (int item = sc; item < SUB * 128; item += TC_SIDE) {
        const int sb = item >> 7, c = item & 127;
        const uint32_t cw = __ldg(tp + sb * 16 + (c >> 3));
        int ed, q;
        const bool valid = e.col_of(cw, c, ed, q);
        float sd = 0.f;
        int mr = dump;
        if (valid) {
          int i, j; float sq;
          const float4 g = edge_geo(ed, i, j, sq);
          const float gv[3] = {g.x, g.y, g.z};
          const bool isz = (sq == 0.f);
          int gslot = 0;
          if (q == 0) {
            sd = isz ? 1.f : sq;
          } else {
            const int k = dirmap(ekind(), q - 1, i, j, dim);
            gslot = 1 + k;
            float acc = 0.f;
#pragma unroll
            for (int cc = 0; cc < 3; ++cc)
              if (cc < dim) acc = fmaf(gv[cc], TCF(xt)[(i * dim + cc) * e.ntan + k] - TCF(xt)[(j * dim + cc) * e.ntan + k], acc);
            sd = isz ? 0.f : 2.f * acc;
          }
          if (want_msg && !((c & 7) == 0 && DIV && !(cw & CH_OWNER))) {
            if (kind == TT_FIRST) {
              const int u = c & 7;
              if (u <= dim) mr = ((i - win_i) * (1 + dim) + u) * U;
              else mr = -(1 + (i * ND + gslot));
            } else if (kind == TT_EDGE1) {
              mr = i * U;
            } else {
              mr = ((i - win_i) * win_ns + (gslot - win_s)) * U;
            }
          }
        }
        TCF(colsd)[(tb * SUB + sb) * 128 + c] = sd;
        TCI(colmrow)[(tb * SUB + sb) * 128 + c] = mr;
      }
      if (sc < 48) {
        const uint32_t w = __ldg(tp + sc);
        if (sc < 32) TCW(chw)[tb * 32 + sc] = w;
        else TCW(hdr)[tb * 16 + (sc - 32)] = w;
      }
    }
    __device__ __forceinline__ void side_coords(int tb, int tile) {
      const KernelArgs& a = e.a;
      const EcnfBlockParams& bp = e.m.blk[b];
      const int sc = e.tid - TC_EPI, n = e.n, dim = e.dim, D = e.D;
      const int ek = ekind();
      const float bpv = bp.bp[0];
      float* cd = TCF(cdbuf);
      const float* pd = TCF(pdh) + tb * 512;
#pragma unroll 1
      for (int item = sc; item < SUB * 128; item += TC_SIDE) {
        const int sb = item >> 7, c = item & 127;
        const uint32_t cw = TCW(chw)[tb * 32 + sb * 16 + (c >> 3)];
        int ed, q;
        const bool valid = e.col_of(cw, c, ed, q);
        float val[3] = {0.f, 0.f, 0.f};
        if (valid) {
          int i, j; float sq;
          const float4 g = edge_geo(ed, i, j, sq);
          const float gv[3] = {g.x, g.y, g.z};
          const bool isz = (sq == 0.f);
          const float len = sqrtf(isz ? 1.f : sq), inv = 1.f / (e.m.C + len);
          const int h2 = c >> 6, cl = c & 63;
          if (q == 0) {
            const float pg = e.full_dot(pd, h2, sb, cl) + bpv;
#pragma unroll
            for (int cc = 0; cc < 3; ++cc) val[cc] = pg * gv[cc] * inv;
          } else {
            const int k = dirmap(ek, q - 1, i, j, dim);
            const float pg = e.full_dot(pd, h2, sb, cl & ~7) + bpv, pdv = e.full_dot(pd, h2, sb, cl);
            const float ld = isz ? 0.f : TCF(colsd)[(tb * SUB + sb) * 128 + c] / (2.f * len);
#pragma unroll
            for (int cc = 0; cc < 3; ++cc) {
              if (cc < dim) {
                const float vc = gv[cc];
                const float vd = TCF(xt)[(i * dim + cc) * e.ntan + k] - TCF(xt)[(j * dim + cc) * e.ntan + k];
                val[cc] = (pdv * vc + pg * vd) * inv - pg * vc * ld * inv * inv;
              }
            }
          }
        }
        cd[(sb * 128 + c) * 3] = val[0]; cd[(sb * 128 + c) * 3 + 1] = val[1]; cd[(sb * 128 + c) * 3 + 2] = val[2];
      }
      e.side_bar();
      const int P = e.hdr(tb, TH_P);
      if constexpr (!DIV) {
        const int i_first = e.hdr(tb, TH_IFIRST), i_last = e.hdr(tb, TH_ILAST);
        const int g0 = ch_gid(TCW(chw)[tb * 32]);
        for (int idx = sc; idx < (i_last - i_first + 1) * dim; idx += TC_SIDE) {
          const int i = i_first + idx / dim, cc = idx % dim;
          const int ea = max(g0, i * (n - 1)), eb = min(g0 + 8 * P, min((i + 1) * (n - 1), e.E));
          float acc = 0.f;
          for (int ed = ea; ed < eb; ++ed) {
            const int lg = ed - g0, pch = lg >> 3;
            const int sb = pch % SUB, col = ((pch / SUB) & 1) * 64 + (pch / (2 * SUB)) * 8 + (lg & 7);
            acc += cd[(sb * 128 + col) * 3 + cc];
          }
          TCF(xacc)[i * dim + cc] += acc;
        }
      } else {
        auto widx = [](int q) { return (q % SUB) * 16 + ((q / SUB) & 1) * 8 + q / (2 * SUB); };
        const int per = 8 * dim;
        if (ek == KIND_FIRST) {
          const int pp = dim * dim;
#pragma unroll 1
          for (int item = sc; item < P * pp; item += TC_SIDE) {
            const int pch = item / pp, rem = item - pch * pp, u = 1 + dim + rem / dim, cc = rem % dim;
            const uint32_t cw = TCW(chw)[tb * 32 + widx(pch)];
            const int ij = __float_as_int(TCF(egv)[ch_gid(cw) * 4 + 3]);
            const int i = ij & 255, j = ij >> 8;
            const int col = (pch % SUB) * 128 + ((pch / SUB) & 1) * 64 + (pch / (2 * SUB)) * 8 + u;
            TCF(xtacc)[(i * dim + cc) * D + j * dim + (u - 1 - dim)] += cd[col * 3 + cc];
          }
        }
        const uint32_t runmask = (uint32_t)e.hdr(tb, TH_RUNMASK);
        const int nruns = __popc(runmask);
#pragma unroll 1
        for (int item = sc; item < nruns * per; item += TC_SIDE) {
          const int ri = item / per, rem = item - ri * per, u = rem / dim, cc = rem - u * dim;
          const int pch = __fns(runmask, 0, ri + 1);
          auto colof = [&](int q) { return (q % SUB) * 128 + ((q / SUB) & 1) * 64 + (q / (2 * SUB)) * 8 + u; };
          const uint32_t cw = TCW(chw)[tb * 32 + widx(pch)];
          if (u >= ch_cnt(cw)) continue;
          const int i = __float_as_int(TCF(egv)[ch_gid(cw) * 4 + 3]) & 255;
          if (ek == KIND_FIRST && u > dim) continue;
          if (u == 0 && !(cw & CH_OWNER)) continue;
          if (ek == KIND_LAST && u > 0 && u - 1 != cc) continue;
          float acc = 0.f;
          int q = pch;
          do {
            acc += cd[colof(q) * 3 + cc];
            --q;
          } while (q >= 0 && !(TCW(chw)[tb * 32 + widx(q)] & CH_RUNEND));
          if (u == 0) TCF(xacc)[i * dim + cc] += acc;
          else if (ek == KIND_LAST) TCF(dacc)[i * dim + cc] += acc;
          else TCF(xtacc)[(i * dim + cc) * e.ntan + (ek == KIND_MID ? ch_qb(cw) + u - 2 : i * dim + (u - 1))] += acc;
        }
      }
      e.side_bar();
    }

    __device__ __forceinline__ void epi(int s, int tb, int tile, int w) {
      const KernelArgs& a = e.a;
      const EcnfBlockParams& bp = e.m.blk[b];
      const int L = e.m.L;
      float v[64];
      e.qbeg();
      if (w == 0) e.wait_bar(B_BUILT, s);
      const float bias = w < L ? bp.be[w][e.fu] : bp.bx[w - L][e.fu];
      {
        uint32_t x[32], y[32];
        e.ld_half_issue(s, 0, x);
        tmem_wait_ld();
        e.ld_half_issue(s, 1, y);
#pragma unroll
        for (int c = 0; c < 32; ++c) v[c] = __uint_as_float(x[c]);
        if (w == 0) e.template act_half<true>(v, 0, bias, tb, wdf);
        else e.template act_half<false>(v, 0, bias, tb, 0.f);
        if (w < NL - 1) e.write_half(s, v, 0, e.f);
        tmem_wait_ld();
#pragma unroll
        for (int c = 0; c < 32; ++c) v[32 + c] = __uint_as_float(y[c]);
      }
      if (w == NL - 1 && tile + 2 < ntiles) e.arrive(B_READY, s);
      if (w == 0) e.template act_half<true>(v, 1, bias, tb, wdf);
      else e.template act_half<false>(v, 1, bias, tb, 0.f);
      if (w < NL - 1) {
        e.write_half(s, v, 1, e.f);
        e.qend(P_EPI);
        if (w == L - 1 && want_msg) { messages(s, tb, v); e.qend(P_MSG); }
      } else {
        e.qend(P_EPI);
        e.warp_dot(v, wpf, TCF(pdh) + tb * 512 + e.warp * 64);
        e.qend(P_HEAD);
      }
    }
    __device__ __forceinline__ void messages(int s, int tb, const float (&v)[64]) {
      const KernelArgs& a = e.a;
      const EcnfBlockParams& bp = e.m.blk[b];
      const int hh = e.hh, lane = e.lane, warp = e.warp, sub = e.sub;
      const float* pd = TCF(pdot) + s * 512;
      e.warp_dot(v, waf, TCF(pdot) + s * 512 + warp * 64);
      e.half_bar();
      {
        const float bav = bp.ba[0];
        float aco[2], bco[2];
        const uint32_t cw = e.my_chw(tb, lane >> 2);
        const float raw[2] = {e.full_dot(pd, hh, sub, 2 * lane), e.full_dot(pd, hh, sub, 2 * lane + 1)};
        float eg[2];
        if constexpr (DIV) {
          const float rawp = __shfl_sync(0xffffffffu, raw[0], lane & ~3);
          eg[0] = eg[1] = fast_sigmoid(rawp + bav);
        } else {
          eg[0] = fast_sigmoid(raw[0] + bav);
          eg[1] = fast_sigmoid(raw[1] + bav);
        }
#pragma unroll
        for (int u2 = 0; u2 < 2; ++u2) {
          const int u = (2 * lane + u2) & 7;
          const bool valid = (cw & CH_VALID) && u < ch_cnt(cw);
          const bool prim = !DIV || u == 0;
          aco[u2] = !valid ? 0.f : (prim ? ((!DIV || (cw & CH_OWNER)) ? eg[u2] : 0.f) : eg[u2]);
          bco[u2] = (!valid || prim) ? 0.f : eg[u2] * (1.f - eg[u2]) * raw[u2];
        }
        *reinterpret_cast<float2*>(TCF(wA) + warp * 64 + 2 * lane) = make_float2(aco[0], aco[1]);
        *reinterpret_cast<float2*>(TCF(wB) + warp * 64 + 2 * lane) = make_float2(bco[0], bco[1]);
      }
      __syncwarp();
      const int nc = e.my_nch(tb);
      float* mac = TCF(macc) + (size_t)(hh * SUB + sub) * (a.lay.mrows + 1) * U + e.fu;
      const float* wa_ = TCF(wA) + warp * 64;
      const int* mr_ = TCI(colmrow) + (tb * SUB + sub) * 128 + 64 * hh;
      if constexpr (!DIV) {
        int cur = mr_[0];
        float acc = 0.f;
#pragma unroll
        for (int c = 0; c < 64; ++c) {
          if (c < 8 * nc) {
            const int mr = mr_[c];
            if (mr != cur) { mac[cur] += acc; acc = 0.f; cur = mr; }
            acc = fmaf(v[c], wa_[c], acc);
          }
        }
        mac[cur] += acc;
      } else {
        const float* wb_ = TCF(wB) + warp * 64;
        const float inv_sqrt_nb = rsqrtf((float)(e.n - 1));
        float2 acc2[4];
#pragma unroll
        for (int k = 0; k < 4; ++k) acc2[k] = make_float2(0.f, 0.f);
#pragma unroll
        for (int ch = 0; ch < 8; ++ch) {
          if (ch < nc) {
            const float2 curm = splat2(v[8 * ch]);
            const float4 wa0 = reinterpret_cast<const float4*>(wa_)[2 * ch], wa1 = reinterpret_cast<const float4*>(wa_)[2 * ch + 1];
            const float4 wb0 = reinterpret_cast<const float4*>(wb_)[2 * ch], wb1 = reinterpret_cast<const float4*>(wb_)[2 * ch + 1];
            const float2 wav[4] = {make_float2(wa0.x, wa0.y), make_float2(wa0.z, wa0.w), make_float2(wa1.x, wa1.y), make_float2(wa1.z, wa1.w)};
            const float2 wbv[4] = {make_float2(wb0.x, wb0.y), make_float2(wb0.z, wb0.w), make_float2(wb1.x, wb1.y), make_float2(wb1.z, wb1.w)};
#pragma unroll
            for (int k = 0; k < 4; ++k) acc2[k] = fma2(col2(v, 8 * ch + 2 * k), wav[k], fma2(curm, wbv[k], acc2[k]));
            if (e.my_chw(tb, ch) & CH_GRPEND) {
              const int4 ma = reinterpret_cast<const int4*>(mr_)[2 * ch], mb = reinterpret_cast<const int4*>(mr_)[2 * ch + 1];
              const int mr[8] = {ma.x, ma.y, ma.z, ma.w, mb.x, mb.y, mb.z, mb.w};
              float old[8];
#pragma unroll
              for (int u = 0; u < 8; ++u) old[u] = mac[mr[u] >= 0 ? mr[u] : a.lay.mrows * U];
#pragma unroll
              for (int k = 0; k < 4; ++k) {
                const float acc[2] = {acc2[k].x, acc2[k].y};
                const float2 sum = add2(make_float2(old[2 * k], old[2 * k + 1]), acc2[k]);
                const float s[2] = {sum.x, sum.y};
#pragma unroll
                for (int j = 0; j < 2; ++j) {
                  const int u = 2 * k + j;
                  if (mr[u] >= 0) mac[mr[u]] = s[j];
                  else e.Mg()[(size_t)(-1 - mr[u]) * U + e.fu] = acc[j] * inv_sqrt_nb;
                }
                acc2[k] = make_float2(0.f, 0.f);
              }
            }
          }
        }
      }
      if (e.hdr(tb, TH_FLUSH)) {
        e.epi_bar();
        const int win_i = e.hdr(tb, TH_WIN_I), win_nr = e.hdr(tb, TH_WIN_NR), win_s = e.hdr(tb, TH_WIN_S), win_ns = e.hdr(tb, TH_WIN_NS);
        const float inv_sqrt_nb = rsqrtf((float)(e.n - 1));
        const size_t cstride = (size_t)(a.lay.mrows + 1) * U;
        float* m0p = TCF(macc) + e.fu;
        constexpr int RG = TC_EPI / U;
        for (int wi = 0; wi < win_nr; ++wi) {
          const int i = win_i + wi;
          for (int ws = e.tid / U; ws < win_ns; ws += RG) {
            const int rr = wi * win_ns + ws;
            const int gslot = (kind == TT_FIRST) ? (ws == 0 ? 0 : 1 + i * e.dim + (ws - 1)) : win_s + ws;
            float sum = 0.f;
#pragma unroll
            for (int cp = 0; cp < 2 * SUB; ++cp) { sum += m0p[cp * cstride + rr * U]; m0p[cp * cstride + rr * U] = 0.f; }
            e.Mg()[((size_t)i * e.ND + gslot) * U + e.fu] = sum * inv_sqrt_nb;
          }
        }
        e.epi_bar();
      }
    }
  };

  __device__ __forceinline__ void eval(float t, const float* xin, const int32_t* feat, float* fout) {
    if (is_epi) {
      if (tid < dim) {
        float s = 0.f;
        for (int i = 0; i < n; ++i) s += xin[i * dim + tid];
        TCF(mu)[tid] = s / (float)n;
      }
      if (tid >= 32 && tid < 32 + m.T / 2) {
        const int k = tid - 32;
        const float arg = (t * 1000.f) * m.freqs[k];
        TCF(tau)[k] = sinf(arg);
        TCF(tau)[k + m.T / 2] = cosf(arg);
      }
      epi_bar();
      for (int i = tid; i < D; i += TC_EPI) {
        const float v = xin[i] - TCF(mu)[i % dim];
        TCF(xs)[i] = v;
        TCF(xs0)[i] = v;
      }
      const float invn = 1.f / (float)n;
      if constexpr (DIV) {
        if (hutch) {
          for (int i = tid; i < D; i += TC_EPI) {
            float mean = 0.f;
            for (int node = 0; node < n; ++node) mean += eps_g[node * dim + i % dim];
            TCF(xt)[i] = eps_g[i] - mean * invn;
          }
        } else {
          for (int idx = tid; idx < D * D; idx += TC_EPI) {
            const int ra = idx / D, k = idx - ra * D;
            const int ia = ra / dim, ca = ra - ia * dim, ik = k / dim, ck = k - ik * dim;
            TCF(xt)[idx] = (ca == ck) ? ((ia == ik ? 1.f : 0.f) - invn) : 0.f;
          }
        }
      }
      float* h0 = hA();
      for (int idx = tid; idx < n * H; idx += TC_EPI) {
        const int node = idx / H, col = idx - node * H;
        int ft = feat[node];
        ft = max(0, min(m.nfeat - 1, ft));
        h0[(size_t)node * ND * H + col] = m.embed[ft * H + col];
      }
      epi_bar();
    }
#pragma unroll 1
    for (int b = 0; b < m.nblocks; ++b) {
      const bool last = (b == m.nblocks - 1);
      const bool htan = DIV && b > 0;
      const int ekind = !DIV ? TT_EDGE1 : hutch ? TT_MID : last ? TT_LAST : (b == 0 ? TT_FIRST : TT_MID);
      const int nkind = DIV ? TT_NODE : TT_NODE1;
      pbeg();
      if (!is_side) {
        const int kind = htan ? TT_NODE : TT_NODE1;
        NodePre p{*this, b, a.tabs.cnt[kind], last ? 1 : 2, kind};
        run_phase(p);
      }
      if (is_epi || is_side) phase_bar();
      pend(P_NODE_PRE);
      {
        EdgePh p{*this, b, a.tabs.cnt[ekind], 2 * m.L, ekind, htan, !last, 0.f, 0.f, 0.f};
        run_phase(p);
      }
      if (is_epi || is_side) phase_bar();
      pend(P_EDGE);
      if (!last && !is_side) {
        NodePost p{*this, b, a.tabs.cnt[nkind], m.L + 1, nkind, htan};
        run_phase(p);
      }
      if (is_epi) {
        epi_bar();
        const float invnb = 1.f / (float)(n - 1);
        for (int i = tid; i < D; i += TC_EPI) TCF(xs)[i] += TCF(xacc)[i] * invnb;
        if (DIV && (!last || hutch))
          for (int i = tid; i < D * ntan; i += TC_EPI) TCF(xt)[i] += TCF(xtacc)[i] * invnb;
      }
      if (is_epi || is_side) phase_bar();
      pend(P_NODE_POST);
    }
    if (is_epi) {
      const float fs = m.final_scaling[0];
      for (int i = tid; i < D; i += TC_EPI) fout[i] = (TCF(xs)[i] - TCF(xs0)[i] - TCF(mu)[i % dim]) * fs;
      if (DIV && tid == 0) {
        float s = 0.f;
        if (hutch) {
          for (int d = 0; d < D; ++d) s = fmaf(eps_g[d], TCF(xt)[d] - eps_g[d], s);
          fout[D] = fs * s;
        } else {
          const float invnb = 1.f / (float)(n - 1);
          for (int d = 0; d < D; ++d) s += TCF(xt)[d * D + d] + TCF(dacc)[d] * invnb;
          fout[D] = fs * (s - (float)D);
        }
      }
    }
    __syncthreads();
  }
};

template <int U, int H, bool DIV, bool SAVE>
__global__ void __launch_bounds__(TC_NT, 1) ecnf_solve_tc_kernel(const __grid_constant__ KernelArgs a) {
  __shared__ long long s_traj;
  __shared__ float s_ctl[8];
  EngineTC<U, H, DIV> eng(a);
  solve_body<EngineTC<U, H, DIV>, DIV, SAVE>(a, eng, s_traj, s_ctl);
  eng.finish(reinterpret_cast<long long*>(reinterpret_cast<char*>(a.counter) + 64));
}

struct TcPrepItem {
  int src_off;
  int dst_off;
  int ksub, N;
  int nsub, lane_stride;
};
constexpr int TC_PREP_MAX = 64;
struct TcPrepList {
  int count;
  TcPrepItem item[TC_PREP_MAX];
};

__global__ void tc_prep_kernel(const float* __restrict__ params, unsigned char* __restrict__ image, const TcPrepList list) {
  const TcPrepItem it = list.item[blockIdx.y];
  uint32_t* dst = reinterpret_cast<uint32_t*>(image + it.dst_off);
  const int K = it.nsub * it.ksub;
  const int words = K / 2;
  for (int idx = blockIdx.x * blockDim.x + threadIdx.x; idx < 128 * words; idx += gridDim.x * blockDim.x) {
    const int wd = idx / 128, lane = idx - wd * 128;
    const int sl = lane / it.lane_stride, o = lane - sl * it.lane_stride;
    const int k0 = 2 * wd, sk = k0 / it.ksub, kk = k0 - sk * it.ksub;
    float x0 = 0.f, x1 = 0.f;
    if (sl == sk && sl < it.nsub && o < it.N) {
      x0 = params[it.src_off + (size_t)kk * it.N + o];
      x1 = params[it.src_off + (size_t)(kk + 1) * it.N + o];
    }
    uint32_t h, l;
    split_pack(x0, x1, h, l);
    const size_t oo = ((size_t)(wd >> 2) * 128 + lane) * 4 + (wd & 3);
    dst[oo] = h;
    dst[(size_t)(K / 8) * 128 * 4 + oo] = l;
  }
}

__global__ void tc_tables_kernel(uint32_t* __restrict__ out, int n, int dim, int SUB, int MR, int ntan, TcTabs tabs) {
  __shared__ uint32_t stage[TC_TILE_WORDS];
  const int k = blockIdx.x;
  if (threadIdx.x == 0 && k < TT_COUNT) tc_pack(k, n, dim, SUB, MR, out + (size_t)tabs.off[k] * TC_TILE_WORDS, ntan, stage);
}

#undef TCF
#undef TCI
#undef TCW

}
```

ecnf_b200/csrc/ecnf_tc.cuh:

```cuda
#pragma once
#include <cuda_bf16.h>
#include <cuda_runtime.h>
#include <stdint.h>

namespace ecnf_tc {

__device__ __forceinline__ uint32_t smem_u32(const void* p) { return (uint32_t)__cvta_generic_to_shared(p); }

__host__ __device__ __forceinline__ int canon_index(int row, int k, int rows) {
  return ((k >> 3) * (rows >> 3) + (row >> 3)) * 64 + (row & 7) * 8 + (k & 7);
}

__device__ __forceinline__ void tmem_alloc(uint32_t* smem_dst, uint32_t ncols) {
  asm volatile("tcgen05.alloc.cta_group::1.sync.aligned.shared::cta.b32 [%0], %1;" ::"r"(smem_u32(smem_dst)), "r"(ncols)
               : "memory");
  asm volatile("tcgen05.relinquish_alloc_permit.cta_group::1.sync.aligned;" ::: "memory");
}
__device__ __forceinline__ void tmem_dealloc(uint32_t taddr, uint32_t ncols) {
  asm volatile("tcgen05.dealloc.cta_group::1.sync.aligned.b32 %0, %1;" ::"r"(taddr), "r"(ncols) : "memory");
}
__device__ __forceinline__ void tc_fence_before() { asm volatile("tcgen05.fence::before_thread_sync;" ::: "memory"); }
__device__ __forceinline__ void tc_fence_after() { asm volatile("tcgen05.fence::after_thread_sync;" ::: "memory"); }
__device__ __forceinline__ void fence_proxy_async() { asm volatile("fence.proxy.async.shared::cta;" ::: "memory"); }

__device__ __forceinline__ void mbar_init(uint64_t* bar, uint32_t count) {
  asm volatile("mbarrier.init.shared::cta.b64 [%0], %1;" ::"r"(smem_u32(bar)), "r"(count) : "memory");
  asm volatile("fence.mbarrier_init.release.cluster;" ::: "memory");
}
__device__ __forceinline__ uint32_t mbar_try_wait(uint64_t* bar, uint32_t parity) {
  uint32_t ok;
  asm volatile(
      "{\n\t"
      ".reg .pred p;\n\t"
      "mbarrier.try_wait.parity.shared::cta.b64 p, [%1], %2;\n\t"
      "selp.u32 %0, 1, 0, p;\n\t"
      "}\n"
      : "=r"(ok)
      : "r"(smem_u32(bar)), "r"(parity)
      : "memory");
  return ok;
}
__device__ __forceinline__ void mbar_wait(uint64_t* bar, uint32_t parity) {
  while (!mbar_try_wait(bar, parity)) {
  }
}
__device__ __forceinline__ void mbar_wait_parked(uint64_t* bar, uint32_t parity, uint32_t ns) {
  uint32_t ok;
  do {
    asm volatile(
        "{\n\t"
        ".reg .pred p;\n\t"
        "mbarrier.try_wait.parity.shared::cta.b64 p, [%1], %2, %3;\n\t"
        "selp.u32 %0, 1, 0, p;\n\t"
        "}\n"
        : "=r"(ok)
        : "r"(smem_u32(bar)), "r"(parity), "r"(ns)
        : "memory");
  } while (!ok);
}
__device__ __forceinline__ void mbar_arrive(uint64_t* bar) {
  asm volatile("mbarrier.arrive.shared::cta.b64 _, [%0];" ::"r"(smem_u32(bar)) : "memory");
}
__device__ __forceinline__ void named_bar_sync(int id, int nthreads) {
  asm volatile("bar.sync %0, %1;" ::"r"(id), "r"(nthreads) : "memory");
}
__device__ __forceinline__ void prefetch_l2_bulk(const void* gsrc, uint32_t bytes) {
  asm volatile("cp.async.bulk.prefetch.L2.global [%0], %1;" ::"l"(gsrc), "r"(bytes) : "memory");
}

__device__ __forceinline__ uint64_t make_sdesc(uint32_t smem_addr, uint32_t lbo_bytes, uint32_t sbo_bytes) {
  return (uint64_t)((smem_addr & 0x3FFFF) >> 4) | ((uint64_t)(lbo_bytes >> 4) << 16) | ((uint64_t)(sbo_bytes >> 4) << 32) |
         ((uint64_t)1 << 46);
}
constexpr uint32_t IDESC_B_MN = 1u << 16;
__host__ __device__ __forceinline__ uint32_t make_idesc_bf16(int m, int n) {
  return (1u << 4) | (1u << 7) | (1u << 10) | ((uint32_t)(n >> 3) << 17) | ((uint32_t)(m >> 4) << 24);
}

__device__ __forceinline__ bool elect_one() {
  uint32_t pred;
  asm volatile(
      "{\n\t"
      ".reg .pred p;\n\t"
      "elect.sync _|p, 0xffffffff;\n\t"
      "selp.u32 %0, 1, 0, p;\n\t"
      "}\n"
      : "=r"(pred));
  return pred != 0;
}

__device__ __forceinline__ void mma_ss(uint32_t d_tmem, uint64_t adesc, uint64_t bdesc, uint32_t idesc, uint32_t accum) {
  asm volatile(
      "{\n\t"
      ".reg .pred p;\n\t"
      "setp.ne.b32 p, %4, 0;\n\t"
      "tcgen05.mma.cta_group::1.kind::f16 [%0], %1, %2, %3, p;\n\t"
      "}\n" ::"r"(d_tmem),
      "l"(adesc), "l"(bdesc), "r"(idesc), "r"(accum)
      : "memory");
}
__device__ __forceinline__ void mma_ts(uint32_t d_tmem, uint32_t a_tmem, uint64_t bdesc, uint32_t idesc, uint32_t accum) {
  asm volatile(
      "{\n\t"
      ".reg .pred p;\n\t"
      "setp.ne.b32 p, %4, 0;\n\t"
      "tcgen05.mma.cta_group::1.kind::f16 [%0], [%1], %2, %3, p;\n\t"
      "}\n" ::"r"(d_tmem),
      "r"(a_tmem), "l"(bdesc), "r"(idesc), "r"(accum)
      : "memory");
}
__device__ __forceinline__ void mma_commit(uint64_t* bar) {
  asm volatile("tcgen05.commit.cta_group::1.mbarrier::arrive::one.shared::cluster.b64 [%0];" ::"r"(smem_u32(bar)) : "memory");
}

__device__ __forceinline__ void tmem_ld32(uint32_t taddr, uint32_t (&v)[32]) {
  asm volatile(
      "tcgen05.ld.sync.aligned.32x32b.x32.b32 "
      "{%0, %1, %2, %3, %4, %5, %6, %7, %8, %9, %10, %11, %12, %13, %14, %15, "
      "%16, %17, %18, %19, %20, %21, %22, %23, %24, %25, %26, %27, %28, %29, %30, %31}, [%32];\n"
      : "=r"(v[0]), "=r"(v[1]), "=r"(v[2]), "=r"(v[3]), "=r"(v[4]), "=r"(v[5]), "=r"(v[6]), "=r"(v[7]), "=r"(v[8]),
        "=r"(v[9]), "=r"(v[10]), "=r"(v[11]), "=r"(v[12]), "=r"(v[13]), "=r"(v[14]), "=r"(v[15]), "=r"(v[16]),
        "=r"(v[17]), "=r"(v[18]), "=r"(v[19]), "=r"(v[20]), "=r"(v[21]), "=r"(v[22]), "=r"(v[23]), "=r"(v[24]),
        "=r"(v[25]), "=r"(v[26]), "=r"(v[27]), "=r"(v[28]), "=r"(v[29]), "=r"(v[30]), "=r"(v[31])
      : "r"(taddr)
      : "memory");
}
__device__ __forceinline__ uint32_t tmem_ld1(uint32_t taddr) {
  uint32_t v;
  asm volatile("tcgen05.ld.sync.aligned.32x32b.x1.b32 {%0}, [%1];\n" : "=r"(v) : "r"(taddr) : "memory");
  return v;
}
__device__ __forceinline__ void tmem_st32(uint32_t taddr, const uint32_t (&v)[32]) {
  asm volatile(
      "tcgen05.st.sync.aligned.32x32b.x32.b32 [%0], "
      "{%1, %2, %3, %4, %5, %6, %7, %8, %9, %10, %11, %12, %13, %14, %15, %16, "
      "%17, %18, %19, %20, %21, %22, %23, %24, %25, %26, %27, %28, %29, %30, %31, %32};\n" ::"r"(taddr),
      "r"(v[0]), "r"(v[1]), "r"(v[2]), "r"(v[3]), "r"(v[4]), "r"(v[5]), "r"(v[6]), "r"(v[7]), "r"(v[8]), "r"(v[9]),
      "r"(v[10]), "r"(v[11]), "r"(v[12]), "r"(v[13]), "r"(v[14]), "r"(v[15]), "r"(v[16]), "r"(v[17]), "r"(v[18]),
      "r"(v[19]), "r"(v[20]), "r"(v[21]), "r"(v[22]), "r"(v[23]), "r"(v[24]), "r"(v[25]), "r"(v[26]), "r"(v[27]),
      "r"(v[28]), "r"(v[29]), "r"(v[30]), "r"(v[31])
      : "memory");
}
__device__ __forceinline__ void tmem_st16(uint32_t taddr, const uint32_t (&v)[16]) {
  asm volatile(
      "tcgen05.st.sync.aligned.32x32b.x16.b32 [%0], "
      "{%1, %2, %3, %4, %5, %6, %7, %8, %9, %10, %11, %12, %13, %14, %15, %16};\n" ::"r"(taddr),
      "r"(v[0]), "r"(v[1]), "r"(v[2]), "r"(v[3]), "r"(v[4]), "r"(v[5]), "r"(v[6]), "r"(v[7]), "r"(v[8]), "r"(v[9]),
      "r"(v[10]), "r"(v[11]), "r"(v[12]), "r"(v[13]), "r"(v[14]), "r"(v[15])
      : "memory");
}
__device__ __forceinline__ void tmem_wait_ld() { asm volatile("tcgen05.wait::ld.sync.aligned;" ::: "memory"); }
__device__ __forceinline__ void tmem_wait_st() { asm volatile("tcgen05.wait::st.sync.aligned;" ::: "memory"); }

__device__ __forceinline__ float2 fma2(float2 x, float2 y, float2 z) {
  float2 d;
  asm("{\n\t.reg .b64 a, b, c, d;\n\t"
      "mov.b64 a, {%2, %3};\n\tmov.b64 b, {%4, %5};\n\tmov.b64 c, {%6, %7};\n\t"
      "fma.rn.f32x2 d, a, b, c;\n\tmov.b64 {%0, %1}, d;\n\t}"
      : "=f"(d.x), "=f"(d.y)
      : "f"(x.x), "f"(x.y), "f"(y.x), "f"(y.y), "f"(z.x), "f"(z.y));
  return d;
}
__device__ __forceinline__ float2 mul2(float2 x, float2 y) {
  float2 d;
  asm("{\n\t.reg .b64 a, b, d;\n\tmov.b64 a, {%2, %3};\n\tmov.b64 b, {%4, %5};\n\tmul.rn.f32x2 d, a, b;\n\tmov.b64 {%0, %1}, d;\n\t}"
      : "=f"(d.x), "=f"(d.y) : "f"(x.x), "f"(x.y), "f"(y.x), "f"(y.y));
  return d;
}
__device__ __forceinline__ float2 add2(float2 x, float2 y) {
  float2 d;
  asm("{\n\t.reg .b64 a, b, d;\n\tmov.b64 a, {%2, %3};\n\tmov.b64 b, {%4, %5};\n\tadd.rn.f32x2 d, a, b;\n\tmov.b64 {%0, %1}, d;\n\t}"
      : "=f"(d.x), "=f"(d.y) : "f"(x.x), "f"(x.y), "f"(y.x), "f"(y.y));
  return d;
}
__device__ __forceinline__ float2 sub2(float2 x, float2 y) {
  float2 d;
  asm("{\n\t.reg .b64 a, b, d;\n\tmov.b64 a, {%2, %3};\n\tmov.b64 b, {%4, %5};\n\tsub.rn.f32x2 d, a, b;\n\tmov.b64 {%0, %1}, d;\n\t}"
      : "=f"(d.x), "=f"(d.y) : "f"(x.x), "f"(x.y), "f"(y.x), "f"(y.y));
  return d;
}
__device__ __forceinline__ float2 splat2(float x) { return make_float2(x, x); }

__device__ __forceinline__ void split_pack(float x0, float x1, uint32_t& hi, uint32_t& lo) {
  const __nv_bfloat162 h = __floats2bfloat162_rn(x0, x1);
  hi = *reinterpret_cast<const uint32_t*>(&h);
  const float2 r = sub2(make_float2(x0, x1), make_float2(__uint_as_float(hi << 16), __uint_as_float(hi & 0xffff0000u)));
  const __nv_bfloat162 l = __floats2bfloat162_rn(r.x, r.y);
  lo = *reinterpret_cast<const uint32_t*>(&l);
}

}
```

Measured before the change: 848.0.

## Specialize warp roles with register reallocation and split weight prefetch into epilogue

Splits the tensor-core kernel into role-specialized paths: only the 256 epilogue threads run the ODE driver loop, while side and MMA warps sit in a follow loop woken by a named-barrier handoff per evaluation. setmaxnreg shifts registers from the side/MMA warpgroup to the epilogue warpgroups, and role checks become compile-time template branches. Block-wide __syncthreads in the solver become epilogue-only barriers. Weight-tile prefetch into TMEM is split into halves interleaved in the epilogue compute to hide global load latency. This adds handoff barrier cost and a risk of spills if the register budgets are too tight.

```diff
diff --git a/ecnf_b200/csrc/ecnf_solve_impl.cuh b/ecnf_b200/csrc/ecnf_solve_impl.cuh
--- a/ecnf_b200/csrc/ecnf_solve_impl.cuh
+++ b/ecnf_b200/csrc/ecnf_solve_impl.cuh
@@ -220,6 +220,8 @@
   __device__ __forceinline__ void set_eps(const float* e) { eps_g = e; }
   __device__ __forceinline__ float* ode_ptr() const { return ode; }
   __device__ __forceinline__ float* red_ptr() const { return red; }
+  static constexpr int ODE_NT = NT;
+  __device__ __forceinline__ void ode_sync() const { __syncthreads(); }
 
   __device__ void rowdot_tile(const float* X, const float* __restrict__ vec, int nrows) {
     const int warp = tid >> 5, lane = tid & 31;
@@ -591,19 +593,19 @@
   enum { PH_VF = 0, PH_F0 = 1, PH_F1 = 2, PH_STAGE = 3 };
 
   auto rms_of_red = [&]() -> float {
-    __syncthreads();
+    eng.ode_sync();
     if (tid == 0) {
       float s = 0.f;
       for (int i = 0; i < S; ++i) s = fmaf(red[i], red[i], s);
       s_ctl[0] = sqrtf(s / (float)S);
     }
-    __syncthreads();
+    eng.ode_sync();
     const float r = s_ctl[0];
-    __syncthreads();
+    eng.ode_sync();
     return r;
   };
   auto base_logp = [&](const float* v) -> float {
-    __syncthreads();
+    eng.ode_sync();
     if (tid == 0) {
       float s = 0.f;
       for (int cdim = 0; cdim < eng.dim; ++cdim) {
@@ -618,17 +620,17 @@
       const float dof = (float)((eng.n - 1) * eng.dim);
       s_ctl[1] = -0.5f * s - 0.5f * dof * 1.8378770664093453f - dof * logf(a.m.base_scale);
     }
-    __syncthreads();
+    eng.ode_sync();
     const float r = s_ctl[1];
-    __syncthreads();
+    eng.ode_sync();
     return r;
   };
 
   for (;;) {
     if (tid == 0) s_traj = (long long)atomicAdd(a.counter, 1u);
-    __syncthreads();
+    eng.ode_sync();
     const long long b = s_traj;
-    __syncthreads();
+    eng.ode_sync();
     if (b >= a.B) break;
     const int32_t* feat = a.feat + b * eng.n;
     const float* xin = a.x_init + b * D;
@@ -644,20 +646,20 @@
     bool at_dtmin = false;
     const float* ein;
     if (vf_mode) {
-      for (int i = tid; i < D; i += Eng::NT) ys[i] = xin[i];
+      for (int i = tid; i < D; i += Eng::ODE_NT) ys[i] = xin[i];
       phase = PH_VF;
       t_eval = a.t_in[b];
       ein = ys;
     } else {
-      for (int i = tid; i < S; i += Eng::NT) y[i] = (i < D) ? xin[i] : 0.f;
+      for (int i = tid; i < S; i += Eng::ODE_NT) y[i] = (i < D) ? xin[i] : 0.f;
       phase = PH_F0;
       t_eval = dir * T0;
       ein = y;
     }
-    __syncthreads();
+    eng.ode_sync();
     if constexpr (SAVE) {
       for (; next_save < a.n_save && a.ts[next_save] <= T0; ++next_save)
-        for (int i = tid; i < S; i += Eng::NT) put(next_save, i, y[i]);
+        for (int i = tid; i < S; i += Eng::ODE_NT) put(next_save, i, y[i]);
     }
     if (DIV && !vf_mode && !reverse) lp0_start = base_logp(y);
 
@@ -667,30 +669,30 @@
       ++n_evals;
       bool begin_step = false;
       if (phase == PH_VF) {
-        for (int i = tid; i < D; i += Eng::NT) a.out_x[b * D + i] = fo[i];
+        for (int i = tid; i < D; i += Eng::ODE_NT) a.out_x[b * D + i] = fo[i];
         if (DIV && tid == 0) a.out_logs[b] = fo[D];
         running = false;
       } else if (phase == PH_F0) {
-        for (int i = tid; i < S; i += Eng::NT) f0[i] = dir * fo[i];
-        __syncthreads();
+        for (int i = tid; i < S; i += Eng::ODE_NT) f0[i] = dir * fo[i];
+        eng.ode_sync();
         if (c.fixed) {
           tnext = clip_to_end(tprev, tprev + fabsf(c.step_size), T1, true);
           begin_step = true;
         } else {
-          for (int i = tid; i < S; i += Eng::NT) red[i] = y[i] / (c.atol + fabsf(y[i]) * c.rtol);
+          for (int i = tid; i < S; i += Eng::ODE_NT) red[i] = y[i] / (c.atol + fabsf(y[i]) * c.rtol);
           const float d0 = rms_of_red();
-          for (int i = tid; i < S; i += Eng::NT) red[i] = f0[i] / (c.atol + fabsf(y[i]) * c.rtol);
+          for (int i = tid; i < S; i += Eng::ODE_NT) red[i] = f0[i] / (c.atol + fabsf(y[i]) * c.rtol);
           d1 = rms_of_red();
           const bool cond = (d0 < 1e-5f) || (d1 < 1e-5f);
           h0 = cond ? 1e-6f : 0.01f * d0 / d1;
-          for (int i = tid; i < S; i += Eng::NT) ys[i] = y[i] + h0 * f0[i];
-          __syncthreads();
+          for (int i = tid; i < S; i += Eng::ODE_NT) ys[i] = y[i] + h0 * f0[i];
+          eng.ode_sync();
           t_eval = dir * (tprev + h0);
           ein = ys;
           phase = PH_F1;
         }
       } else if (phase == PH_F1) {
-        for (int i = tid; i < S; i += Eng::NT) red[i] = (dir * fo[i] - f0[i]) / (c.atol + fabsf(y[i]) * c.rtol);
+        for (int i = tid; i < S; i += Eng::ODE_NT) red[i] = (dir * fo[i] - f0[i]) / (c.atol + fabsf(y[i]) * c.rtol);
         const float d2 = rms_of_red() / h0;
         const float md = fmaxf(d1, d2);
         const float h1 = (md <= 1e-15f) ? fmaxf(1e-6f, h0 * 1e-3f) : powf(0.01f / md, 1.f / c.error_order);
@@ -698,8 +700,8 @@
         tnext = clip_to_end(tprev, tprev + dt0, T1, true);
         begin_step = true;
       } else {
-        for (int i = tid; i < S; i += Eng::NT) kk[stage * S + i] = (dir * fo[i]) * dt;
-        __syncthreads();
+        for (int i = tid; i < S; i += Eng::ODE_NT) kk[stage * S + i] = (dir * fo[i]) * dt;
+        eng.ode_sync();
         if (stage < 6) {
           ++stage;
         } else {
@@ -709,7 +711,7 @@
             new_prev = tnext;
             new_next = tnext + dt;
           } else {
-            for (int i = tid; i < S; i += Eng::NT) {
+            for (int i = tid; i < S; i += Eng::ODE_NT) {
               float e = 0.f;
               for (int j = 0; j < 7; ++j) {
                 const float bj = c_BERR[j];
@@ -736,7 +738,7 @@
               const float tau_s = a.ts[next_save];
               const bool at_end = !(tau_s < tnext);
               const float sx = (tau_s - tprev) / dt;
-              for (int i = tid; i < S; i += Eng::NT) {
+              for (int i = tid; i < S; i += Eng::ODE_NT) {
                 const float y0 = y[i], y1 = ys[i];
                 float v = y1;
                 if (!at_end) {
@@ -756,10 +758,10 @@
             }
           }
           if (keep) {
-            for (int i = tid; i < S; i += Eng::NT) { y[i] = ys[i]; f0[i] = dir * fo[i]; }
+            for (int i = tid; i < S; i += Eng::ODE_NT) { y[i] = ys[i]; f0[i] = dir * fo[i]; }
             ++n_acc;
           }
-          __syncthreads();
+          eng.ode_sync();
           tprev = new_prev;
           tnext = new_next;
           ++n_steps;
@@ -770,14 +772,14 @@
       }
       if (begin_step) {
         dt = tnext - tprev;
-        for (int i = tid; i < S; i += Eng::NT) kk[i] = f0[i] * dt;
-        __syncthreads();
+        for (int i = tid; i < S; i += Eng::ODE_NT) kk[i] = f0[i] * dt;
+        eng.ode_sync();
         stage = 1;
         phase = PH_STAGE;
         if (c.max_steps <= 0) { status = 1; running = false; }
       }
       if (running && phase == PH_STAGE) {
-        for (int i = tid; i < S; i += Eng::NT) {
+        for (int i = tid; i < S; i += Eng::ODE_NT) {
           float v = y[i];
           for (int j = 0; j < stage; ++j) {
             const float aj = c_A[stage][j];
@@ -785,18 +787,18 @@
           }
           ys[i] = v;
         }
-        __syncthreads();
+        eng.ode_sync();
         t_eval = dir * (tprev + c_C[stage] * dt);
         ein = ys;
       }
     }
-    if (vf_mode) { __syncthreads(); continue; }
+    if (vf_mode) { eng.ode_sync(); continue; }
     if constexpr (SAVE) {
       const int left = a.n_save - next_save;
-      for (int idx = tid; idx < left * S; idx += Eng::NT) put(next_save + idx / S, idx % S, __int_as_float(0x7fffffff));
-    }
-
-    for (int i = tid; i < D; i += Eng::NT) a.out_x[b * D + i] = y[i];
+      for (int idx = tid; idx < left * S; idx += Eng::ODE_NT) put(next_save + idx / S, idx % S, __int_as_float(0x7fffffff));
+    }
+
+    for (int i = tid; i < D; i += Eng::ODE_NT) a.out_x[b * D + i] = y[i];
     float lpb_end = 0.f;
     if (DIV && reverse) lpb_end = base_logp(y);
     if (tid == 0) {
@@ -817,7 +819,7 @@
         }
       }
     }
-    __syncthreads();
+    eng.ode_sync();
   }
 }
 
diff --git a/ecnf_b200/csrc/ecnf_solve_tc.cuh b/ecnf_b200/csrc/ecnf_solve_tc.cuh
--- a/ecnf_b200/csrc/ecnf_solve_tc.cuh
+++ b/ecnf_b200/csrc/ecnf_solve_tc.cuh
@@ -8,9 +8,11 @@
 
 constexpr int TC_NT = 384;
 constexpr int TC_EPI = 256, TC_SIDE = 96;
-#ifndef TC_WPREFETCH
-#define TC_WPREFETCH 0
-#endif
+constexpr int TC_REG_LAUNCH = 168, TC_REG_EPI = 208, TC_REG_WG2 = 88;
+static_assert(2 * TC_REG_EPI + TC_REG_WG2 <= 3 * TC_REG_LAUNCH, "register budgets exceed the launch allocation");
+static_assert(TC_REG_EPI % 8 == 0 && TC_REG_WG2 % 8 == 0, "setmaxnreg budgets are multiples of 8");
+constexpr int TC_BAR_HANDOFF = 6;
+enum { TC_CTL_EXIT = 0, TC_CTL_EVAL = 1 };
 constexpr int TC_BOP = 65536;
 constexpr uint32_t TC_LBO = 128, TC_SBO = 2048;
 constexpr uint32_t TC_LBO_K = 2048, TC_SBO_K = 128;
@@ -250,10 +252,12 @@
   const int n, dim, D, ntan, ND, E;
   const float* eps_g;
   const int tid, f, hh, warp, lane, sub, fu;
-  const bool is_epi, is_side;
   uint32_t tmem;
   uint32_t lane_addr;
   uint32_t par;
+  uint32_t round;
+
+  enum Role { R_EPI, R_SIDE, R_MMA };
 
   enum { B_READY = 0, B_DONE = 1, B_BUILT = 2, B_HEADS = 3, B_BFREE = 4 };
   enum { P_NODE_PRE, P_EDGE, P_NODE_POST, P_WAIT, P_EPI, P_MSG, P_HEAD, P_WLOAD, P_SIDE_WAIT, P_SIDE_GATHER, P_SIDE_COORD,
@@ -277,6 +281,7 @@
   __device__ __forceinline__ float* red_ptr() const { return TCF(red); }
   __device__ __forceinline__ uint64_t* bar(int kind, int s) const { return reinterpret_cast<uint64_t*>(smem_tc + a.lay.bars) + kind * 2 + s; }
   __device__ __forceinline__ uint32_t* tmem_slot() const { return reinterpret_cast<uint32_t*>(smem_tc + a.lay.bars + 96); }
+  __device__ __forceinline__ int* ctl_slot() const { return reinterpret_cast<int*>(smem_tc + a.lay.bars + 104); }
   __device__ __forceinline__ float* hA() const { return a.scratch + (size_t)blockIdx.x * a.scratch_stride; }
   __device__ __forceinline__ float* hB() const { return hA() + (size_t)n * ND * H; }
   __device__ __forceinline__ float* Mg() const { return hB() + (size_t)n * ND * H; }
@@ -287,8 +292,7 @@
       : a(a_), m(a_.m), img(a_.img), hutch(DIV && a_.eps != nullptr), n(a_.m.n), dim(a_.m.dim), D(a_.m.n * a_.m.dim),
         ntan(DIV ? (a_.eps != nullptr ? 1 : a_.m.n * a_.m.dim) : 0), ND(1 + (DIV ? (a_.eps != nullptr ? 1 : a_.m.n * a_.m.dim) : 0)),
         E(a_.m.n * (a_.m.n - 1)), eps_g(nullptr), tid(threadIdx.x), f(threadIdx.x & 127), hh((threadIdx.x >> 7) & 1), warp(threadIdx.x >> 5),
-        lane(threadIdx.x & 31), sub((threadIdx.x & 127) / U_), fu((threadIdx.x & 127) % U_), is_epi(threadIdx.x < TC_EPI),
-        is_side(threadIdx.x >= TC_EPI && threadIdx.x < TC_EPI + TC_SIDE) {
+        lane(threadIdx.x & 31), sub((threadIdx.x & 127) / U_), fu((threadIdx.x & 127) % U_) {
     if (tid == 0) {
       mbar_init(bar(B_READY, 0), TC_EPI); mbar_init(bar(B_READY, 1), TC_EPI);
       mbar_init(bar(B_DONE, 0), 1); mbar_init(bar(B_DONE, 1), 1);
@@ -307,7 +311,8 @@
     tmem = *tmem_slot();
     lane_addr = (uint32_t)(32 * (warp & 3)) << 16;
     par = 0;
-    if (is_epi) {
+    round = 0;
+    if (tid < TC_EPI) {
       uint32_t z[32];
 #pragma unroll
       for (int c = 0; c < 32; ++c) z[c] = 0u;
@@ -315,7 +320,7 @@
       for (int q = 0; q < 4; ++q) tmem_st32(tmem + lane_addr + 128u * hh + 32u * q, z);
       tmem_wait_st();
     }
-    if (is_side)
+    if (tid >= TC_EPI && tid < TC_EPI + TC_SIDE)
       for (int k = tid - TC_EPI; k < ROWB / 4; k += TC_SIDE) reinterpret_cast<uint32_t*>(Himg() + (size_t)n * ND * ROWB)[k] = 0u;
     tc_fence_before();
     __syncthreads();
@@ -487,47 +492,43 @@
     else return p4[(2 * sb) * 64] + p4[(2 * sb + 1) * 64];
   }
   template <int K>
-  __device__ __forceinline__ void fetch_w(int img_off, uint32_t (&wv)[2][K / 4]) {
+  __device__ __forceinline__ void fetch_w(int img_off, int p, uint32_t (&wv)[K / 4]) {
     constexpr int NC = K / 16;
     const uint4* src = reinterpret_cast<const uint4*>(img.base + img_off);
 #pragma unroll
-    for (int p = 0; p < 2; ++p)
-#pragma unroll
-      for (int j = 0; j < NC; ++j) {
-        const uint4 q = __ldg(src + (size_t)(p * (K / 8) + hh * NC + j) * 128 + f);
-        wv[p][4 * j] = q.x; wv[p][4 * j + 1] = q.y; wv[p][4 * j + 2] = q.z; wv[p][4 * j + 3] = q.w;
-      }
+    for (int j = 0; j < NC; ++j) {
+      const uint4 q = __ldg(src + (size_t)(p * (K / 8) + hh * NC + j) * 128 + f);
+      wv[4 * j] = q.x; wv[4 * j + 1] = q.y; wv[4 * j + 2] = q.z; wv[4 * j + 3] = q.w;
+    }
   }
   template <int K>
-  __device__ __forceinline__ void store_w(const uint32_t (&wv)[2][K / 4], uint32_t col) {
-#pragma unroll
-    for (int p = 0; p < 2; ++p) {
-      const uint32_t addr = tmem + col + lane_addr + (uint32_t)(p * (K / 2) + hh * (K / 4));
-      if constexpr (K == 128) tmem_st32(addr, wv[p]);
-      else tmem_st16(addr, wv[p]);
-    }
-    tmem_wait_st();
+  __device__ __forceinline__ void store_w(const uint32_t (&wv)[K / 4], uint32_t col, int p) {
+    const uint32_t addr = tmem + col + lane_addr + (uint32_t)(p * (K / 2) + hh * (K / 4));
+    if constexpr (K == 128) tmem_st32(addr, wv);
+    else tmem_st16(addr, wv);
   }
   template <int K>
   __device__ __forceinline__ void load_w(int img_off, uint32_t col) {
-    constexpr int NC = K / 16;
     uint32_t wv[2][K / 4];
-    const uint4* src = reinterpret_cast<const uint4*>(img.base + img_off);
-#pragma unroll
-    for (int p = 0; p < 2; ++p)
-#pragma unroll
-      for (int j = 0; j < NC; ++j) {
-        const uint4 q = __ldg(src + (size_t)(p * (K / 8) + hh * NC + j) * 128 + f);
-        wv[p][4 * j] = q.x; wv[p][4 * j + 1] = q.y; wv[p][4 * j + 2] = q.z; wv[p][4 * j + 3] = q.w;
-      }
-#pragma unroll
-    for (int p = 0; p < 2; ++p) {
-      const uint32_t addr = tmem + col + lane_addr + (uint32_t)(p * (K / 2) + hh * (K / 4));
-      if constexpr (K == 128) tmem_st32(addr, wv[p]);
-      else tmem_st16(addr, wv[p]);
-    }
+    fetch_w<K>(img_off, 0, wv[0]);
+    fetch_w<K>(img_off, 1, wv[1]);
+    store_w<K>(wv[0], col, 0);
+    store_w<K>(wv[1], col, 1);
     tmem_wait_st();
   }
+  struct WPrefetch {
+    EngineTC& e;
+    const bool on;
+    const int off;
+    const uint32_t col;
+    uint32_t wv[32];
+    __device__ __forceinline__ void fetch(int p) { if (on) e.template fetch_w<128>(off, p, wv); }
+    __device__ __forceinline__ void store(int p) {
+      if (on) { e.qbeg(); e.template store_w<128>(wv, col, p); tmem_wait_st(); e.qend(P_WLOAD); }
+    }
+    __device__ __forceinline__ void mid() { store(0); fetch(1); }
+    __device__ __forceinline__ void end() { store(1); }
+  };
 
   __device__ __forceinline__ const uint32_t* tile_ptr(int kind, int tile) const {
     return a.tabs.base + (size_t)(a.tabs.off[kind] + tile) * TC_TILE_WORDS;
@@ -541,20 +542,18 @@
     return valid;
   }
 
-  template <class P>
+  template <int R, class P>
   __device__ __forceinline__ void run_phase(P& p) {
     const int ntiles = p.ntiles, NL = p.NL;
     const int npairs = (ntiles + 1) >> 1;
     const int total_q = npairs * NL;
-    if (is_epi || (P::side_build && is_side)) p.prologue();
-    if (is_epi && p.stream) {
+    if constexpr (R == R_EPI || (P::side_build && R == R_SIDE)) p.template prologue<R>();
+    if constexpr (R == R_EPI && P::stream) {
       load_w<128>(p.wimg(0), TC_WCOL);
       if (total_q > 1) load_w<128>(p.wimg(1 % NL), TC_WCOL + 128);
     }
-    if constexpr (P::side_build) {
-      if (is_epi || is_side) phase_bar();
-    }
-    if (is_side) {
+    if constexpr (P::side_build && R != R_MMA) phase_bar();
+    if constexpr (R == R_SIDE) {
       if constexpr (P::side_build) {
 #pragma unroll 1
         for (int t0 = 0; t0 < 2 && t0 < ntiles; ++t0) {
@@ -601,7 +600,7 @@
 #pragma unroll 1
     for (int s = 0; s < 2; ++s) {
       if (s >= ntiles) continue;
-      if (is_epi) {
+      if constexpr (R == R_EPI) {
         if constexpr (!P::side_build) { p.build(s, tb_of(s, s), s); arrive(B_READY, s); }
       } else {
         issue_mma(s, tb_of(s, s), first_kind, p.a_col(0, 0), p.K(0), P::side_build, false);
@@ -619,18 +618,13 @@
           const bool last_slot = (s == 1) || (tile + 1 >= ntiles);
           const int ntile = tile + 2;
           const int tb = tb_of(s, tile);
-          if (is_epi) {
-            const bool do_w = p.stream && last_slot && q + 2 < total_q;
-#if TC_WPREFETCH
-            uint32_t wv[2][32];
-            if (do_w) fetch_w<128>(p.wimg((w + 2) % NL), wv);
+          if constexpr (R == R_EPI) {
+            const bool do_w = P::stream && last_slot && q + 2 < total_q;
+            WPrefetch wp{*this, do_w, do_w ? p.wimg((w + 2) % NL) : 0, TC_WCOL + 128u * (q & 1)};
             wait_done(s);
-            if (do_w) { qbeg(); store_w<128>(wv, TC_WCOL + 128 * (q & 1)); qend(P_WLOAD); }
-#else
-            wait_done(s);
-            if (do_w) { qbeg(); load_w<128>(p.wimg((w + 2) % NL), TC_WCOL + 128 * (q & 1)); qend(P_WLOAD); }
-#endif
-            p.epi(s, tb, tile, w);
+            wp.fetch(0);
+            p.epi(s, tb, tile, w, wp);
+            wp.end();
             if (w < NL - 1) arrive(B_READY, s);
             else if constexpr (P::side_build) arrive(B_HEADS, s);
             else if (ntile < ntiles) { p.build(s, tb_of(s, ntile), ntile); arrive(B_READY, s); }
@@ -672,6 +666,7 @@
     __device__ __forceinline__ uint32_t a_col(int, int w) const { return TC_WCOL + 64u * w; }
     __device__ __forceinline__ int K(int) const { return KN; }
     __device__ __forceinline__ int wimg(int) const { return 0; }
+    template <int R>
     __device__ __forceinline__ void prologue() {
       const KernelArgs& a = e.a;
       const EcnfBlockParams& bp = e.m.blk[b];
@@ -702,7 +697,7 @@
       }
       e.qend(P_NBUILD);
     }
-    __device__ __forceinline__ void epi(int s, int tb, int, int w) {
+    __device__ __forceinline__ void epi(int s, int tb, int, int w, WPrefetch&) {
       const KernelArgs& a = e.a;
       const EcnfBlockParams& bp = e.m.blk[b];
       float v[64];
@@ -750,6 +745,7 @@
     static constexpr bool side_build = false;
     __device__ __forceinline__ uint32_t a_col(int q, int) const { return TC_WCOL + 128u * (q & 1); }
     __device__ __forceinline__ int K(int) const { return 128; }
+    template <int R>
     __device__ __forceinline__ void prologue() {}
     __device__ __forceinline__ int wimg(int w) const {
       const TcImgBlock& ib = e.img.blk[b];
@@ -775,7 +771,7 @@
       e.write_B(s, v, e.f);
       e.qend(P_NBUILD);
     }
-    __device__ __forceinline__ void epi(int s, int tb, int, int w) {
+    __device__ __forceinline__ void epi(int s, int tb, int, int w, WPrefetch& wp) {
       const KernelArgs& a = e.a;
       const EcnfBlockParams& bp = e.m.blk[b];
       const int L = e.m.L;
@@ -800,13 +796,16 @@
           for (int u = 0; u < 16; ++u) v[cb + u] += pv[u];
         }
         e.template act_rule<false>(v, 0.f, tb, 0.f);
+        wp.mid();
         e.write_B(s, v, e.f);
       } else if (w < L) {
         const float bias = bp.bh[w][e.fu];
         e.ld_acc(s, v);
         e.template act_rule<false>(v, bias, tb, 0.f);
+        wp.mid();
         e.write_B(s, v, e.f);
       } else {
+        wp.mid();
         if (e.fu >= H) return;
         const float bias = bp.bh[L][e.fu];
         const float* hin = e.hB() + e.fu;
@@ -849,12 +848,13 @@
       const int L = e.m.L;
       return w == 0 ? ib.We0 : (w < L ? ib.We[w] : ib.Wx[w - L]);
     }
+    template <int R>
     __device__ __forceinline__ void prologue() {
       const KernelArgs& a = e.a;
       const EcnfBlockParams& bp = e.m.blk[b];
       const int n = e.n, dim = e.dim, D = e.D;
       constexpr int NTH = TC_EPI + TC_SIDE;
-      if (e.is_epi) {
+      if constexpr (R == R_EPI) {
         wdf = bp.We[0][(size_t)2 * H * U + e.fu];
         waf = bp.wa[e.fu];
         wpf = bp.wp[e.fu];
@@ -1065,7 +1065,7 @@
       e.side_bar();
     }
 
-    __device__ __forceinline__ void epi(int s, int tb, int tile, int w) {
+    __device__ __forceinline__ void epi(int s, int tb, int tile, int w, WPrefetch& wp) {
       const KernelArgs& a = e.a;
       const EcnfBlockParams& bp = e.m.blk[b];
       const int L = e.m.L;
@@ -1083,6 +1083,7 @@
         if (w == 0) e.template act_half<true>(v, 0, bias, tb, wdf);
         else e.template act_half<false>(v, 0, bias, tb, 0.f);
         if (w < NL - 1) e.write_half(s, v, 0, e.f);
+        wp.mid();
         tmem_wait_ld();
 #pragma unroll
         for (int c = 0; c < 32; ++c) v[32 + c] = __uint_as_float(y[c]);
@@ -1210,8 +1211,31 @@
     }
   };
 
+  static constexpr int ODE_NT = TC_EPI;
+  __device__ __forceinline__ void ode_sync() const { epi_bar(); }
+  __device__ __forceinline__ void handoff(int ctl) {
+    if (tid == 0) ctl_slot()[round & 1] = ctl;
+    named_bar_arrive(TC_BAR_HANDOFF, TC_NT);
+    ++round;
+  }
+  template <int R>
+  __device__ __forceinline__ void follow() {
+#pragma unroll 1
+    for (;;) {
+      named_bar_sync(TC_BAR_HANDOFF, TC_NT);
+      const int ctl = ctl_slot()[round & 1];
+      ++round;
+      if (ctl == TC_CTL_EXIT) break;
+      eval_role<R>(0.f, nullptr, nullptr, nullptr);
+    }
+  }
   __device__ __forceinline__ void eval(float t, const float* xin, const int32_t* feat, float* fout) {
-    if (is_epi) {
+    handoff(TC_CTL_EVAL);
+    eval_role<R_EPI>(t, xin, feat, fout);
+  }
+  template <int R>
+  __device__ __forceinline__ void eval_role(float t, const float* xin, const int32_t* feat, float* fout) {
+    if constexpr (R == R_EPI) {
       if (tid < dim) {
         float s = 0.f;
         for (int i = 0; i < n; ++i) s += xin[i * dim + tid];
@@ -1261,34 +1285,36 @@
       const int ekind = !DIV ? TT_EDGE1 : hutch ? TT_MID : last ? TT_LAST : (b == 0 ? TT_FIRST : TT_MID);
       const int nkind = DIV ? TT_NODE : TT_NODE1;
       pbeg();
-      if (!is_side) {
+      if constexpr (R != R_SIDE) {
         const int kind = htan ? TT_NODE : TT_NODE1;
         NodePre p{*this, b, a.tabs.cnt[kind], last ? 1 : 2, kind};
-        run_phase(p);
-      }
-      if (is_epi || is_side) phase_bar();
+        run_phase<R>(p);
+      }
+      if constexpr (R != R_MMA) phase_bar();
       pend(P_NODE_PRE);
       {
         EdgePh p{*this, b, a.tabs.cnt[ekind], 2 * m.L, ekind, htan, !last, 0.f, 0.f, 0.f};
-        run_phase(p);
-      }
-      if (is_epi || is_side) phase_bar();
+        run_phase<R>(p);
+      }
+      if constexpr (R != R_MMA) phase_bar();
       pend(P_EDGE);
-      if (!last && !is_side) {
-        NodePost p{*this, b, a.tabs.cnt[nkind], m.L + 1, nkind, htan};
-        run_phase(p);
-      }
-      if (is_epi) {
+      if constexpr (R != R_SIDE) {
+        if (!last) {
+          NodePost p{*this, b, a.tabs.cnt[nkind], m.L + 1, nkind, htan};
+          run_phase<R>(p);
+        }
+      }
+      if constexpr (R == R_EPI) {
         epi_bar();
         const float invnb = 1.f / (float)(n - 1);
         for (int i = tid; i < D; i += TC_EPI) TCF(xs)[i] += TCF(xacc)[i] * invnb;
         if (DIV && (!last || hutch))
           for (int i = tid; i < D * ntan; i += TC_EPI) TCF(xt)[i] += TCF(xtacc)[i] * invnb;
       }
-      if (is_epi || is_side) phase_bar();
+      if constexpr (R != R_MMA) phase_bar();
       pend(P_NODE_POST);
     }
-    if (is_epi) {
+    if constexpr (R == R_EPI) {
       const float fs = m.final_scaling[0];
       for (int i = tid; i < D; i += TC_EPI) fout[i] = (TCF(xs)[i] - TCF(xs0)[i] - TCF(mu)[i % dim]) * fs;
       if (DIV && tid == 0) {
@@ -1302,17 +1328,28 @@
           fout[D] = fs * (s - (float)D);
         }
       }
-    }
-    __syncthreads();
+      epi_bar();
+    }
   }
 };
 
 template <int U, int H, bool DIV, bool SAVE>
 __global__ void __launch_bounds__(TC_NT, 1) ecnf_solve_tc_kernel(const __grid_constant__ KernelArgs a) {
+  using Eng = EngineTC<U, H, DIV>;
   __shared__ long long s_traj;
   __shared__ float s_ctl[8];
-  EngineTC<U, H, DIV> eng(a);
-  solve_body<EngineTC<U, H, DIV>, DIV, SAVE>(a, eng, s_traj, s_ctl);
+  Eng eng(a);
+  if (threadIdx.x >= TC_EPI) {
+    reg_dealloc<TC_REG_WG2>();
+    if (threadIdx.x < TC_EPI + TC_SIDE) eng.template follow<Eng::R_SIDE>();
+    else eng.template follow<Eng::R_MMA>();
+    reg_alloc<TC_REG_LAUNCH>();
+  } else {
+    reg_alloc<TC_REG_EPI>();
+    solve_body<Eng, DIV, SAVE>(a, eng, s_traj, s_ctl);
+    eng.handoff(TC_CTL_EXIT);
+    reg_dealloc<TC_REG_LAUNCH>();
+  }
   eng.finish(reinterpret_cast<long long*>(reinterpret_cast<char*>(a.counter) + 64));
 }
 
diff --git a/ecnf_b200/csrc/ecnf_tc.cuh b/ecnf_b200/csrc/ecnf_tc.cuh
--- a/ecnf_b200/csrc/ecnf_tc.cuh
+++ b/ecnf_b200/csrc/ecnf_tc.cuh
@@ -64,6 +64,19 @@
 __device__ __forceinline__ void named_bar_sync(int id, int nthreads) {
   asm volatile("bar.sync %0, %1;" ::"r"(id), "r"(nthreads) : "memory");
 }
+__device__ __forceinline__ void named_bar_arrive(int id, int nthreads) {
+  asm volatile("bar.arrive %0, %1;" ::"r"(id), "r"(nthreads) : "memory");
+}
+template <int R>
+__device__ __forceinline__ void reg_alloc() {
+  static_assert(R % 8 == 0 && R >= 24 && R <= 256, "setmaxnreg budget");
+  asm volatile("setmaxnreg.inc.sync.aligned.u32 %0;" ::"n"(R));
+}
+template <int R>
+__device__ __forceinline__ void reg_dealloc() {
+  static_assert(R % 8 == 0 && R >= 24 && R <= 256, "setmaxnreg budget");
+  asm volatile("setmaxnreg.dec.sync.aligned.u32 %0;" ::"n"(R));
+}
 __device__ __forceinline__ void prefetch_l2_bulk(const void* gsrc, uint32_t bytes) {
   asm volatile("cp.async.bulk.prefetch.L2.global [%0], %1;" ::"l"(gsrc), "r"(bytes) : "memory");
 }
```

Result: faster. 856.9 (median of 6 runs) (+1.1%).
